# marbl/Winnowmap

Hardware: AMD Instinct MI355X
Metric: mapped Gbp/s (higher is better)
Workload: dtype int8

## Files before the change

### __graft_entry__.py

```python
import os
import sys

ROOT = os.path.dirname(os.path.abspath(__file__))
sys.path.insert(0, ROOT)
sys.path.insert(0, os.path.join(ROOT, "tests"))


def build():
    from winnowmap_amd import build as b
    b.build_gpu(verbose=True)
    b.build_oracle()
    b.build_emu()
    b.build_emu_selfmap()
    b.build_emu_chain()
    b.build_harness()
    import winnowmap_amd
    from winnowmap_amd import gpu
    gpu.lib()


def smoke():
    import numpy as np
    from winnowmap_amd import gpu
    import wmtest as W
    import kswcases
    ctx = gpu.Context(0, 2 << 30)
    cases = kswcases.ont_segments(5, 64)
    sc = gpu.KswScore(2, -4, -1, 4, 2, 24, 1)
    jobs, seqs = gpu.pack_jobs([(c["q"], c["t"], dict(w=c["w"], zdrop=c["zdrop"], end_bonus=c["end_bonus"], flag=c["flag"])) for c in cases])
    res, pool = ctx.ksw_batch(sc, jobs, seqs)
    for i, c in enumerate(cases):
        o = W.o_ksw_extd2(c["q"], c["t"], w=c["w"], zdrop=c["zdrop"], end_bonus=c["end_bonus"], flag=c["flag"])
        assert all(int(res[i][k]) == o[k] for k in W.EZ_FIELDS), (i, res[i], o)
        assert np.array_equal(pool[res[i]["cig_off"]:res[i]["cig_off"] + res[i]["n_cigar"]], o["cigar"]), i
    import ctypes as C
    import tempfile
    from winnowmap_amd import build as b, synth
    tmp = tempfile.mkdtemp()
    ref = synth.make_reference(1, 200000, 5, repeat_frac=0.1)
    fa = os.path.join(tmp, "ref.fa")
    synth.write_fasta(fa, ref)
    km, cnt = synth.repetitive_kmers(ref, 15)
    kf = os.path.join(tmp, "rep.txt")
    synth.write_kmer_list(kf, km, cnt, 15)
    reads, _ = synth.make_reads(ref, 4, 12000, 6, profile="ont", sv_frac=0.25)
    rs = [synth.codes_to_ascii(r) for r in reads]
    idx = gpu.Index(fa, kf, k=15, w=50, n_threads=4)
    idx.upload(ctx)
    m = gpu.Mapper(ctx, idx, "map-ont", gpu.MM_F_CIGAR | gpu.MM_F_OUT_CG)
    text, hits, cigars, first = m.map(["r%d" % i for i in range(len(rs))], rs)
    H = C.CDLL(b.build_harness())
    H.h_index_build.restype = C.c_void_p
    H.h_index_build.argtypes = [C.c_char_p, C.c_char_p, C.c_int, C.c_int, C.c_int]
    H.h_map_many.argtypes = [C.c_void_p, C.c_char_p, C.c_int64, C.c_int, C.POINTER(C.c_char_p), W.i32p, C.c_int, W.i32p, C.c_int, C.POINTER(C.c_int64), W.u32p, C.c_int64, C.POINTER(C.c_int64)]
    hh = H.h_index_build(fa.encode(), kf.encode(), 15, 50, 4)
    n = len(rs)
    ho = np.zeros(16 * 1024, np.int32); co = np.zeros(4000000, np.uint32); hf = (C.c_int64 * (n + 1))(); nc = C.c_int64()
    nh = H.h_map_many(hh, b"map-ont", 0x4 | 0x20, n, (C.c_char_p * n)(*rs), np.array([len(r) for r in rs], np.int32), 2, ho, 1024, hf, co, len(co), C.byref(nc))
    assert nh == len(hits) and nh > 0, (nh, len(hits))
    assert np.array_equal(ho[:16 * nh].reshape(-1, 16), hits) and np.array_equal(co[:nc.value], cigars) and list(hf) == list(first)
    m.close(); idx.close(); ctx.close()
    print("smoke OK: %d ksw alignments and %d end-to-end hits (%d CIGAR ops) bit-exact vs the oracle" % (len(cases), nh, nc.value))


if __name__ == "__main__":
    build()
    if len(sys.argv) > 1 and sys.argv[1] == "smoke":
        smoke()
```

### include/wm_gpu.h

```cpp
#ifndef WM_GPU_H
#define WM_GPU_H
#include <stdint.h>
#include <stddef.h>
#ifdef __cplusplus
extern "C" {
#endif

#define WM_OK        0
#define WM_ENODEV   (-1)
#define WM_EINVAL   (-2)
#define WM_ENOMEM   (-3)
#define WM_EINTERNAL (-4)

typedef struct wm_ctx_s wm_ctx_t;

typedef struct { uint64_t x, y; } wm128_t;

int wm_ctx_create(int device, size_t arena_bytes, wm_ctx_t **out);
void wm_ctx_destroy(wm_ctx_t *ctx);
const char *wm_last_error(void);
const char *wm_build_defines(void);
int wm_device_count(void);
float wm_last_kernel_ms(const wm_ctx_t *ctx);
int wm_ctx_device(const wm_ctx_t *ctx);

typedef struct {
	int8_t match, mismatch, sc_ambi;
	int8_t q, e, q2, e2;
} wm_ksw_score_t;

typedef struct {
	uint32_t q_off, t_off;
	int32_t qlen, tlen;
	int32_t w, zdrop, end_bonus, flag;
} wm_ksw_job_t;

typedef struct {
	int32_t max, zdropped, max_q, max_t, mqe, mqe_t, mte, mte_q, score, reach_end;
	int32_t n_cigar;
	uint32_t cig_off;
} wm_ksw_result_t;

int wm_ksw_batch(wm_ctx_t *ctx, const wm_ksw_score_t *sc, int n_jobs, const wm_ksw_job_t *jobs,
                 const uint8_t *seqs, size_t seqs_bytes,
                 wm_ksw_result_t *results, uint32_t *cigar_pool, size_t cigar_cap, size_t *cigar_used);

typedef struct {
	int64_t qwin_off;
	int32_t qwin_len, q_pos;
	int32_t rid, t_pos;
	int32_t qlen, tlen;
	int32_t w, zdrop, end_bonus, flag;
	int8_t step, has_n, pad[6];
} wm_ksw_pos_t;
int wm_reads_upload(wm_ctx_t *ctx, const uint8_t *codes, size_t n);
int wm_ksw_batch_pos(wm_ctx_t *ctx, const wm_ksw_score_t *sc, int n_jobs, const wm_ksw_pos_t *jobs,
                     wm_ksw_result_t *results, uint32_t *cigar_pool, size_t cigar_cap, size_t *cigar_used);
#define WM_KSW_F_ZDWALK 0x10000
typedef struct { int32_t max_zdrop, t0, t1, q0, q1; } wm_zd_t;
int wm_ksw_batch_pos_zd(wm_ctx_t *ctx, const wm_ksw_score_t *sc, int n_jobs, const wm_ksw_pos_t *jobs,
                        wm_ksw_result_t *results, uint32_t *cigar_pool, size_t cigar_cap, size_t *cigar_used, wm_zd_t *zd);

int wm_debug_stripe_timing(uint64_t *out16, int reset);

int wm_ksw_ll_i16(int qlen, const uint8_t *query, int tlen, const uint8_t *target, const int8_t *mat5x5, int gapo, int gape, int *qe, int *te);

int wm_ksw_exts2_batch(wm_ctx_t *ctx, const wm_ksw_score_t *sc, int noncan, int junc_bonus, int n_jobs, const wm_ksw_job_t *jobs,
                       const uint8_t *seqs, size_t seqs_bytes, const uint8_t *junc,
                       wm_ksw_result_t *results, uint32_t *cigar_pool, size_t cigar_cap, size_t *cigar_used);

typedef struct wm_ksw_dev_batch_s wm_ksw_dev_batch_t;
int wm_ksw_dev_prepare(wm_ctx_t *ctx, const wm_ksw_score_t *sc, int n_jobs, const wm_ksw_job_t *jobs,
                       const uint8_t *seqs, size_t seqs_bytes, wm_ksw_dev_batch_t **out);
int wm_ksw_dev_run(wm_ctx_t *ctx, wm_ksw_dev_batch_t *b);
int wm_ksw_dev_fetch(wm_ctx_t *ctx, wm_ksw_dev_batch_t *b, wm_ksw_result_t *results,
                     uint32_t *cigar_pool, size_t cigar_cap, size_t *cigar_used);
int wm_ksw_dev_stats(const wm_ksw_dev_batch_t *b, uint64_t *cells, uint64_t *tb_bytes, float *dp_ms, float *bt_ms);
void wm_ksw_dev_free(wm_ctx_t *ctx, wm_ksw_dev_batch_t *b);

void wm_ksw_set_routing(int on, int rows4, int rows8);
void wm_ksw_set_chain_routing(int mode, int min_rows_exact, int bp);
void wm_ksw_set_dual(int on);
int wm_ksw_dual_enabled(void);

int wm_ksw_extd2(wm_ctx_t *ctx, int qlen, const uint8_t *query, int tlen, const uint8_t *target, int8_t m,
                 const int8_t *mat, int8_t q, int8_t e, int8_t q2, int8_t e2, int w, int zdrop, int end_bonus,
                 int flag, wm_ksw_result_t *ez, uint32_t **cigar_out);

typedef struct wm_index_s wm_index_t;
int wm_index_build(const char *fasta, const char *kmer_file, int k, int w, int n_threads, wm_index_t **out);
int wm_index_build_gpu(wm_ctx_t *ctx, const char *fasta, const char *kmer_file, int k, int w, int n_threads, wm_index_t **out, double *stats);
int wm_index_build_flag(const char *fasta, const char *kmer_file, int k, int w, int idx_flag, int n_threads, wm_index_t **out);
int wm_index_build_gpu_flag(wm_ctx_t *ctx, const char *fasta, const char *kmer_file, int k, int w, int idx_flag, int n_threads, wm_index_t **out, double *stats);
void wm_index_destroy(wm_index_t *idx);
int wm_index_save(const wm_index_t *idx, const char *path);
int wm_index_load(const char *path, const char *kmer_file, wm_index_t **out);
int wm_index_upload(wm_ctx_t *ctx, const wm_index_t *idx);
int wm_index_read_junc_bed(wm_index_t *idx, const char *path);
int wm_index_add_junc(wm_index_t *idx, int ctg, int n, const int32_t *st, const int32_t *en, const int32_t *strand);
int wm_index_n_seq(const wm_index_t *idx);
const char *wm_index_seq_name(const wm_index_t *idx, int rid);
int wm_index_seq_len(const wm_index_t *idx, int rid);
uint64_t wm_index_n_minimizers(const wm_index_t *idx);
const uint64_t *wm_index_get(const wm_index_t *idx, uint64_t minier, int *n);

int wm_write_repetitive_kmers(const char *fasta, int k, double distinct, const char *out_path, uint64_t *n_out);
int wm_write_repetitive_kmers_gpu(wm_ctx_t *ctx, const char *fasta, int k, double distinct, const char *out_path, uint64_t *n_out, double *stats);
int wm_index_export(const wm_index_t *idx, uint64_t *sizes9, uint32_t *S, uint64_t *hkey, uint64_t *hval, uint64_t *P, uint8_t *bloom,
                    uint64_t *seq_meta, char *names);
int wm_index_import(const uint64_t *sizes9, const uint32_t *S, const uint64_t *hkey, const uint64_t *hval, const uint64_t *P, const uint8_t *bloom,
                    const uint64_t *seq_meta, const char *names, wm_index_t **out);

int wm_sketch_batch(wm_ctx_t *ctx, int n, const uint8_t *seqs, size_t seqs_bytes, const uint64_t *seq_off, const int32_t *len,
                    wm128_t *out, size_t out_cap, uint64_t *out_off, int32_t *counts);
int wm_sketch_set_filter(wm_ctx_t *ctx, const uint8_t *bits, size_t n_bytes, uint64_t table_bits, uint32_t salt0, uint32_t salt1, int k, int w);
int wm_seed_batch(wm_ctx_t *ctx, int n, const wm128_t *mini, const uint64_t *mini_off, const int32_t *n_mini, const int32_t *qlen,
                  int max_occ, int64_t flag, wm128_t *out, size_t out_cap, uint64_t *out_off, int32_t *n_anchors, int32_t *rep_len);
typedef struct { uint32_t lo, eq; } wm_qkey_t;
int wm_index_query_key(const wm_index_t *idx, const char *qname, wm_qkey_t *key);
int wm_seed_batch_keyed(wm_ctx_t *ctx, int n, const wm128_t *mini, const uint64_t *mini_off, const int32_t *n_mini, const int32_t *qlen, const wm_qkey_t *keys,
                        int max_occ, int64_t flag, wm128_t *out, size_t out_cap, uint64_t *out_off, int32_t *n_anchors, int32_t *rep_len);
typedef struct { int32_t max_dist_x, min_dist_x, max_dist_y, bw, max_skip, max_iter, min_cnt, min_sc; float gap_scale;
                 int32_t is_cdna;  } wm_chain_par_t;
int wm_chain_batch(wm_ctx_t *ctx, int n, wm128_t *a, const uint64_t *a_off, const int32_t *n_a, const wm_chain_par_t *par,
                   uint64_t *u, uint64_t *u_off, int32_t *n_u, int32_t *n_v);
typedef struct {
	int64_t seq_off;
	uint64_t stage_off, pre_off;
	int32_t len, n_pre;
	wm_chain_par_t par;
} wm_window_job_t;
typedef struct { int32_t n_anchors, rep_len, n_mini, n_u, n_v; uint32_t u_off, a_off; } wm_window_res_t;
int wm_window_batch(wm_ctx_t *ctx, int n, const wm_window_job_t *jobs, const uint8_t *seqs, size_t seqs_bytes, const wm128_t *pre, size_t n_pre_total,
                    int max_occ, int64_t flag, wm_window_res_t *res, uint64_t *u_pool, size_t u_cap, size_t *u_used, wm128_t *a_pool, size_t a_cap, size_t *a_used);
int wm_window_batch_keyed(wm_ctx_t *ctx, int n, const wm_window_job_t *jobs, const wm_qkey_t *keys, const uint8_t *seqs, size_t seqs_bytes, const wm128_t *pre, size_t n_pre_total,
                          int max_occ, int64_t flag, wm_window_res_t *res, uint64_t *u_pool, size_t u_cap, size_t *u_used, wm128_t *a_pool, size_t a_cap, size_t *a_used);
float wm_last_aux_ms(const wm_ctx_t *ctx);

typedef struct wm_mapper_s wm_mapper_t;
int wm_mapper_create(wm_ctx_t *ctx, const wm_index_t *idx, const char *preset, int64_t flag, wm_mapper_t **out);
void wm_mapper_destroy(wm_mapper_t *m);
int wm_mapper_set_threads(wm_mapper_t *m, int n_threads, size_t arena_bytes_per_group);
int wm_map_reads(wm_mapper_t *m, int n, const char *const *names, const char *const *seqs, const int32_t *lens,
                 const char **text, size_t *text_len, const int32_t **hits, const uint32_t **cigars, const int64_t **hit_first);
#define WM_MAX_SLOTS 4
int wm_map_reads_slot(wm_mapper_t *m, int slot, int n, const char *const *names, const char *const *seqs, const int32_t *lens,
                      const char **text, size_t *text_len, const int32_t **hits, const uint32_t **cigars, const int64_t **hit_first);
int wm_mapper_set_slots(wm_mapper_t *m, int n);
int wm_map_reads_rep_len_defined(const wm_mapper_t *m, int slot, const uint8_t **flags, size_t *n);
int wm_map_file(wm_mapper_t *m, const char *reads_path, const char *out_path, int64_t mini_batch_bases, double *stats);
int wm_index_upload_dev(wm_ctx_t *ctx, const wm_index_t *idx, const void *d_S, const void *d_hkey, const void *d_hval, const void *d_P, const void *d_bloom, int src_device);
int wm_index_upload_peer(wm_ctx_t *dst, const wm_index_t *idx, const wm_ctx_t *src);
int wm_map_file_multi(wm_mapper_t *const *mappers, int n, const char *reads_path, const char *out_path, int64_t mini_batch_bases, double *stats);
int wm_mapper_set_cmdline(wm_mapper_t *m, int argc, const char *const *argv);
int wm_set_cmdline(int argc, const char *const *argv);
typedef struct {
	int64_t flag;
	int32_t seed, sdust_thres, max_qlen;
	int32_t bw, max_gap, max_gap_ref, min_gap_ref, max_frag_len;
	int32_t max_chain_skip, max_chain_iter, min_cnt, min_chain_score;
	float chain_gap_scale;
	int32_t SVaware, SVawareMinReadLength, suffixSampleOffset, min_mapq;
	float min_qcov;
	int32_t minPrefixLength, maxPrefixLength;
	float prefixIncrementFactor;
	int32_t stage2_bw, stage2_zdrop_inv, stage2_max_gap;
	float mask_level;
	int32_t mask_len;
	float pri_ratio;
	int32_t best_n;
	int32_t max_join_long, max_join_short, min_join_flank_sc;
	float min_join_flank_ratio, alt_drop;
	int32_t a, b, q, e, q2, e2, sc_ambi;
	int32_t zdrop, zdrop_inv, end_bonus, min_dp_max, min_ksw_len;
	float max_clip_ratio;
	float mid_occ_frac;
	int32_t min_mid_occ, mid_occ, max_occ;
	int64_t mini_batch_size, max_sw_mat;
	int32_t noncan, junc_bonus;
	int32_t anchor_ext_len, anchor_ext_shift;
} wm_mapopt_t;
int wm_mapopt_preset(const char *preset, wm_mapopt_t *out, int *k, int *w);
int wm_mapper_create_opt(wm_ctx_t *ctx, const wm_index_t *idx, const wm_mapopt_t *opt, wm_mapper_t **out);
int wm_index_build_parts(const char *fasta, const char *kmer_file, int k, int w, int n_threads, uint64_t batch_bases, wm_index_t **out, int cap, int *n_parts);
int wm_map_file_split(wm_ctx_t *ctx, int n_parts, wm_index_t *const *parts, const wm_mapopt_t *opt, int n_threads, const char *reads_path, const char *out_path,
                      int64_t mini_batch_bases, double *stats);
typedef struct wm_split_s wm_split_t;
int wm_split_begin(wm_ctx_t *ctx, const wm_mapopt_t *opt, int k, int w, int n_threads, const char *reads_path, int64_t mini_batch_bases, wm_split_t **out);
int wm_split_add_part(wm_split_t *s, wm_index_t *part);
int wm_split_finish(wm_split_t *s, const char *out_path, double *stats);
void wm_split_abort(wm_split_t *s);
int wm_map_file_split_fasta(wm_ctx_t *ctx, const char *fasta, const char *kmer_file, int k, int w, int build_threads, uint64_t batch_bases, int on_device,
                            const wm_mapopt_t *opt, int n_threads, const char *reads_path, const char *out_path, int64_t mini_batch_bases, double *stats, int *n_parts);

int wm_mapper_set_sam_header(wm_mapper_t *m, int on);
int wm_mapper_stats(const wm_mapper_t *m, uint64_t *out9);
int wm_mapper_kernel_stats(const wm_mapper_t *m, double *out, int cap, int *n_classes);
int wm_ksw_n_classes(void);
int wm_mapper_kernel_union(const wm_mapper_t *m, double since_ms, double *out, int cap, double *now_ms);
int wm_mapper_host_stats(const wm_mapper_t *m, double *out, int cap);
int wm_sam_header(const wm_index_t *idx, int argc, const char *const *argv, const char **text, size_t *text_len);

#ifdef __cplusplus
}
#endif
#endif
```

### winnowmap_amd/build.py

```python
import os
import subprocess
import sys

HERE = os.path.dirname(os.path.abspath(__file__))
ROOT = os.path.dirname(HERE)
CSRC = os.path.join(HERE, "csrc")
LIB = os.path.join(HERE, "libwmgpu.so")
HIPCC = os.environ.get("HIPCC", "/opt/rocm/bin/hipcc")


class _Lock:

    def __init__(self, target):
        self.path = target + ".lock"

    def __enter__(self):
        import fcntl
        self.f = open(self.path, "w")
        fcntl.flock(self.f, fcntl.LOCK_EX)

    def __exit__(self, *a):
        import fcntl
        fcntl.flock(self.f, fcntl.LOCK_UN)
        self.f.close()


def _run_to(target, cmd_for):
    tmp = target + ".tmp%d" % os.getpid()
    try:
        subprocess.check_call(cmd_for(tmp))
        os.replace(tmp, target)
    finally:
        if os.path.exists(tmp):
            os.unlink(tmp)


def _newer(target, sources):
    if not os.path.exists(target):
        return True
    t = os.path.getmtime(target)
    return any(os.path.getmtime(s) > t for s in sources)


HIP_FLAGS = ["--offload-arch=gfx950", "-O3", "-std=c++17", "-ffp-contract=off", "-Wno-unused-value", "-mllvm", "-disable-promote-alloca-to-vector"]


UNITS = ("wm_rt", "wm_ksw", "wm_index", "wm_window", "wm_mapper")


def build_gpu(force=False, verbose=False, out=None):
    global LIB
    if out is not None:
        saved, LIB = LIB, out
        try:
            return build_gpu(force, verbose)
        finally:
            LIB = saved
    srcs = [os.path.join(d, f) for d, _, fs in os.walk(CSRC) for f in fs if ".obj" not in d] + [os.path.join(ROOT, "include", "wm_gpu.h")]
    defines = " ".join(os.environ.get("WM_KERNEL_DEFINES", "").split())
    stamp = LIB + ".defines"
    with _Lock(LIB):
        have = open(stamp).read() if os.path.exists(stamp) else ""
        if not force and not _newer(LIB, srcs) and have == defines:
            return LIB
        defs = ["-D" + d for d in defines.split()] + ['-DWM_BUILD_DEFINES="%s"' % defines]
        objdir = os.path.join(CSRC, ".obj", os.path.basename(LIB))
        os.makedirs(objdir, exist_ok=True)
        cmds = [[HIPCC] + HIP_FLAGS + defs + ["-fPIC", "-c", os.path.join(CSRC, u + ".hip"), "-o", os.path.join(objdir, u + ".o")] for u in UNITS]
        if verbose:
            for c in cmds:
                print(" ".join(c), file=sys.stderr)
        procs = [subprocess.Popen(c) for c in cmds]
        rcs = [p.wait() for p in procs]
        if any(rcs):
            raise subprocess.CalledProcessError(next(r for r in rcs if r), cmds[next(i for i, r in enumerate(rcs) if r)])
        link = lambda out_: [HIPCC, "--offload-arch=gfx950", "-shared", "-fPIC", "-o", out_] + [os.path.join(objdir, u + ".o") for u in UNITS] + ["-lz", "-lpthread"]
        if verbose:
            print(" ".join(link(LIB)), file=sys.stderr)
        _run_to(LIB, link)
        with open(stamp, "w") as f:
            f.write(defines)
    return LIB


def build_oracle():
    with _Lock(os.path.join(ROOT, "oracle", "libwm_oracle.so")):
        subprocess.check_call(["make", "-C", os.path.join(ROOT, "oracle"), "oracle"], stdout=subprocess.DEVNULL)
        if os.path.exists("/root/reference/src/map.c"):
            subprocess.check_call(["make", "-C", os.path.join(ROOT, "oracle"), "ref", "-j8"], stdout=subprocess.DEVNULL)
            if os.path.exists(LIB):
                subprocess.check_call(["make", "-C", os.path.join(ROOT, "oracle"), "wm", "subst", "-j8"], stdout=subprocess.DEVNULL)


def build_emu(defines=()):
    emu = os.path.join(ROOT, "tests", "simt_emu")
    tag = "".join("_" + "".join(ch if ch.isalnum() else "_" for ch in d) for d in defines)
    out = os.path.join(emu, "libwm_emu%s.so" % tag)
    srcs = [os.path.join(emu, f) for f in ("emu_driver.cpp", "simt.h")] + [os.path.join(CSRC, f) for f in os.listdir(CSRC) if f.endswith(".h")]
    with _Lock(out):
        if _newer(out, srcs):
            _run_to(out, lambda o: ["g++", "-O1", "-std=c++17", "-fPIC", "-shared", "-ffp-contract=off", "-Wno-unknown-pragmas"] +
                    ["-D" + d for d in defines] + ["-I" + emu, "-I" + CSRC, "-o", o, os.path.join(emu, "emu_driver.cpp")])
    return out


def build_emu_selfmap():
    emu = os.path.join(ROOT, "tests", "simt_emu")
    out = os.path.join(emu, "libwm_emu_selfmap.so")
    srcs = [os.path.join(emu, f) for f in ("emu_selfmap.cpp", "simt.h")] + \
           [os.path.join(CSRC, f) for f in ("seedchain_kernel.h", "window_kernel.h", "wm_internal.h", os.path.join("host", "wm_names.h"))]
    with _Lock(out):
        if _newer(out, srcs):
            _run_to(out, lambda o: ["g++", "-O1", "-std=c++17", "-fPIC", "-shared", "-ffp-contract=off", "-Wno-unknown-pragmas",
                                    "-I" + emu, "-I" + CSRC, "-o", o, os.path.join(emu, "emu_selfmap.cpp")])
    return out


def build_emu_stripe(defines=()):
    emu = os.path.join(ROOT, "tests", "simt_emu")
    tag = "".join("_" + "".join(ch if ch.isalnum() else "_" for ch in d) for d in defines)
    out = os.path.join(emu, "libwm_emu_stripe%s.so" % tag)
    srcs = [os.path.join(emu, f) for f in ("emu_stripe.cpp", "simt.h")] + \
           [os.path.join(CSRC, f) for f in ("ksw_stripe_kernel.h", "ksw_packed_kernel.h", "ksw_kernel.h", "ksw_plan.h")]
    with _Lock(out):
        if _newer(out, srcs):
            _run_to(out, lambda o: ["g++", "-O1", "-std=c++17", "-fPIC", "-shared", "-pthread", "-ffp-contract=off", "-Wno-unknown-pragmas"] +
                    ["-D" + d for d in defines] + ["-I" + emu, "-I" + CSRC, "-o", o, os.path.join(emu, "emu_stripe.cpp")])
    return out


def build_emu_chain(defines=()):
    emu = os.path.join(ROOT, "tests", "simt_emu")
    tag = "".join("_" + "".join(ch if ch.isalnum() else "_" for ch in d) for d in defines)
    out = os.path.join(emu, "libwm_emu_chain%s.so" % tag)
    srcs = [os.path.join(emu, f) for f in ("emu_chain.cpp", "simt.h")] + \
           [os.path.join(CSRC, f) for f in ("ksw_chain_kernel.h", "ksw_stripe_kernel.h", "ksw_packed_kernel.h", "ksw_kernel.h", "ksw_plan.h")]
    with _Lock(out):
        if _newer(out, srcs):
            _run_to(out, lambda o: ["g++", "-O1", "-std=c++17", "-fPIC", "-shared", "-pthread", "-ffp-contract=off", "-Wno-unknown-pragmas"] +
                    ["-D" + d for d in defines] + ["-I" + emu, "-I" + CSRC, "-o", o, os.path.join(emu, "emu_chain.cpp")])
    return out


def build_harness():
    hd = os.path.join(ROOT, "tests", "host_harness")
    out = os.path.join(hd, "libwm_harness.so")
    srcs = [os.path.join(hd, "harness.cpp"), os.path.join(ROOT, "oracle", "wm_oracle.c")] + \
           [os.path.join(CSRC, "host", f) for f in os.listdir(os.path.join(CSRC, "host"))]
    with _Lock(out):
        if _newer(out, srcs):
            _run_to(out, lambda o: ["g++", "-std=c++17", "-O2", "-g", "-ffp-contract=off", "-fPIC", "-shared", "-o", o,
                                    os.path.join(hd, "harness.cpp"), os.path.join(ROOT, "oracle", "wm_oracle.c"), "-lz", "-pthread"])
    return out


if __name__ == "__main__":
    build_gpu(force="--force" in sys.argv, verbose=True)
    build_oracle()
    build_emu()
    build_emu_selfmap()
    build_emu_stripe()
    build_emu_chain()
    build_harness()
```

### winnowmap_amd/csrc/wm_ksw.hip

```cpp
#include "wm_rt.h"
#include "simt.h"
#include "ksw_kernel.h"
#include "ksw_packed_kernel.h"
#include "ksw_packed_multi_kernel.h"
#include "ksw_dual_kernel.h"
#include "ksw_stripe_kernel.h"
#include "ksw_chain_kernel.h"
#include "ksw_exts2_kernel.h"
#include "cigar_walk.h"
#include "reads2bit.h"

#ifndef WM_OCC_HINT
#define WM_OCC_HINT 1
#endif
template <int BP, bool CLIP, bool HASN, bool EXACT>
__global__ __launch_bounds__(64, (WM_OCC_HINT && BP == 8 && CLIP && EXACT) ? 4 : 1) void ksw_dpp_kernel(wm_ksw_score_t sc, const wm_ksw_djob_t *__restrict__ jobs,
                                                      const int *__restrict__ order, const uint8_t *__restrict__ seqs,
                                                      uint8_t *__restrict__ tb, wm_ksw_dres_t *__restrict__ res)
{
	if constexpr (EXACT || CLIP || BP >= 16) WM_SETPRIO(2);
	const int j = order[blockIdx.x];
	wmk::ksw_dp_packed<BP, CLIP, HASN, EXACT>(sc, jobs[j], seqs, tb, res + j);
}

__global__ __launch_bounds__(64) void ksw_generic_kernel(wm_ksw_score_t sc, const wm_ksw_djob_t *__restrict__ jobs, const int *__restrict__ order,
                                                          const uint8_t *__restrict__ seqs, uint8_t *__restrict__ tb, uint8_t *scratch,
                                                          const uint64_t *__restrict__ scratch_off, wm_ksw_dres_t *__restrict__ res)
{
	WM_SETPRIO(3);
	const int j = order[blockIdx.x];
	const wm_ksw_djob_t jb = jobs[j];
	const int T = (jb.tlen + 15) / 16 * 16;
	signed char *mem = (signed char*)(scratch + scratch_off[blockIdx.x]);
	int *Hm = (int*)(mem + (size_t)8 * T);
	wmk::ksw_dp_generic<true>(sc, jb, seqs, tb, mem, Hm, res + j);
}

template <int K, int WN>
__global__ __launch_bounds__(64 * WM_KSW_BLK_NWV) void ksw_block_kernel(wm_ksw_score_t sc, const wm_ksw_djob_t *__restrict__ jobs, const int *__restrict__ order,
                                                                         const uint8_t *__restrict__ seqs, uint8_t *__restrict__ tb, wm_ksw_dres_t *__restrict__ res, int seq_cap,
                                                                         int *gstate, const uint64_t *__restrict__ gstate_off)
{
	WM_SETPRIO(3);
	extern __shared__ __attribute__((aligned(16))) unsigned char smem[];
	constexpr bool GLOBAL = WN == 0;
	const int j = order[blockIdx.x];
	const wm_ksw_djob_t jb = jobs[j];
	const int wn = GLOBAL ? (int)wm_ksw_blk3_wn(jb.tlen) : WN;
	int *W0 = GLOBAL ? gstate + gstate_off[blockIdx.x] : (int*)smem, *W1 = W0 + wn, *Hm = W1 + wn;
	int *pub = GLOBAL ? (int*)smem : Hm + wn;
	uint8_t *sq = (uint8_t*)(pub + WM_KSW_BLK_PUB);
	const int qpad = (jb.qlen + 15) & ~15;
	if (qpad + jb.tlen <= seq_cap) {
		uint8_t *st = sq + qpad;
		for (int i = threadIdx.x; i < jb.qlen; i += blockDim.x) sq[i] = seqs[jb.q_off + i];
		for (int i = threadIdx.x; i < jb.tlen; i += blockDim.x) st[i] = seqs[jb.t_off + i];
		__syncthreads();
		wmk::ksw_dp_block<WM_KSW_BLK_NWV, K, GLOBAL>(sc, jb, sq, st, tb, W0, W1, Hm, wn, pub, res + j);
	} else
		wmk::ksw_dp_block<WM_KSW_BLK_NWV, K, GLOBAL>(sc, jb, seqs + jb.q_off, seqs + jb.t_off, tb, W0, W1, Hm, wn, pub, res + j);
}

template <int BP, int NWV, bool CLIP = true, bool HASN = true>
__global__ __launch_bounds__(64 * NWV) void ksw_pmulti_kernel(wm_ksw_score_t sc, const wm_ksw_djob_t *__restrict__ jobs, const int *__restrict__ order,
                                                                         const uint8_t *__restrict__ seqs, uint8_t *__restrict__ tb, wm_ksw_dres_t *__restrict__ res, int seq_cap)
{
	WM_SETPRIO(3);
	extern __shared__ __attribute__((aligned(16))) unsigned char smem[];
	typedef wmk::ksw_pmulti_lds<BP, NWV> L;
	int *lds = (int*)smem;
	uint8_t *sq = (uint8_t*)(lds + L::INTS);
	const int j = order[blockIdx.x];
	const wm_ksw_djob_t jb = jobs[j];
	const int qpad = (jb.qlen + 15) & ~15;
	if (qpad + jb.tlen <= seq_cap) {
		uint8_t *st = sq + qpad;
		for (int i = threadIdx.x; i < jb.qlen; i += blockDim.x) sq[i] = seqs[jb.q_off + i];
		for (int i = threadIdx.x; i < jb.tlen; i += blockDim.x) st[i] = seqs[jb.t_off + i];
		__syncthreads();
		if (jb.flag & KSW_F_APPROX_MAX) wmk::ksw_dp_pmulti<BP, NWV, CLIP, HASN, false>(sc, jb, sq, st, tb, lds, res + j);
		else wmk::ksw_dp_pmulti<BP, NWV, CLIP, HASN, true>(sc, jb, sq, st, tb, lds, res + j);
	} else {
		const uint8_t *qp = seqs + jb.q_off, *tp = seqs + jb.t_off;
		if (jb.flag & KSW_F_APPROX_MAX) wmk::ksw_dp_pmulti<BP, NWV, CLIP, HASN, false>(sc, jb, qp, tp, tb, lds, res + j);
		else wmk::ksw_dp_pmulti<BP, NWV, CLIP, HASN, true>(sc, jb, qp, tp, tb, lds, res + j);
	}
}

template <int BP, int NWV, bool CLIP, bool HASN>
__global__ __launch_bounds__(64 * NWV) void ksw_stripe_kernel(wm_ksw_score_t sc, const wm_ksw_djob_t *__restrict__ jobs, const int *__restrict__ order,
                                                               const uint8_t *__restrict__ seqs, uint8_t *__restrict__ tb, wm_ksw_dres_t *__restrict__ res)
{
	WM_SETPRIO(WM_STRIPE_PRIO);
	__shared__ int lds[wmk::ksw_stripe_lds<BP, NWV>::INTS];
	const int j = order[blockIdx.x];
	const wm_ksw_djob_t jb = jobs[j];
	if (jb.flag & KSW_F_APPROX_MAX) wmk::ksw_dp_stripe<BP, NWV, CLIP, HASN, false>(sc, jb, seqs, tb, lds, res + j);
	else wmk::ksw_dp_stripe<BP, NWV, CLIP, HASN, true>(sc, jb, seqs, tb, lds, res + j);
}

template <int BP, bool CLIP, bool HASN, bool EXACT>
__global__ __launch_bounds__(64, (WM_OCC_HINT && BP == 2 && EXACT) ? 4 : 1) void ksw_chain_kernel(wm_ksw_score_t sc, const wm_ksw_djob_t *__restrict__ jobs, const int *__restrict__ order,
                                                        const uint8_t *__restrict__ seqs, uint8_t *__restrict__ tb, wm_ksw_dres_t *__restrict__ res,
                                                        const uint4 *__restrict__ cmap, int *ticket, wm_mbox_t *mail)
{
	WM_SETPRIO(WM_STRIPE_PRIO);
	__shared__ int tbs[wm_chain_box::GROUP * 32 * BP];
	int tk = 0;
	if (threadIdx.x == 0) tk = atomicAdd(ticket, 1);
	tk = __builtin_amdgcn_readfirstlane(tk);
	const uint4 m = cmap[tk];
	const int j = order[m.x];
	const wm_ksw_djob_t jb = jobs[j];
	wm_mbox_t *mb = mail + (size_t)m.z * 16;
	wmk::ksw_dp_chain<BP, CLIP, HASN, EXACT>(sc, jb, seqs, tb, mb, (int)m.w, (int)m.y, tbs, res + j);
}

__global__ __launch_bounds__(256) void ksw_reset_kernel(int n, const wm_ksw_djob_t *__restrict__ jobs, wm_ksw_dres_t *__restrict__ res)
{
	const int j = blockIdx.x * 256 + threadIdx.x;
	if (j >= n || jobs[j].klass >= 0) return;
	wm_ksw_dres_t z;
	z.max = 0; z.zdropped = 0; z.max_q = z.max_t = z.mqe_t = z.mte_q = -1; z.score = z.mqe = z.mte = KSW_NEG_INF; z.reach_end = 0; z.n_cigar = 0; z.bt_i = z.bt_j = -1;
	res[j] = z;
}

__global__ __launch_bounds__(64) void ksw_expand_kernel(const wm_ksw_djob_t *__restrict__ jobs, const wm_ksw_dsrc_t *__restrict__ src,
                                                         const uint64_t *__restrict__ reads_pk, const uint64_t *__restrict__ reads_nm, const uint32_t *__restrict__ S,
                                                         uint8_t *__restrict__ seqs)
{
	WM_SETPRIO(1);
	const int j = blockIdx.x;
	const wm_ksw_djob_t jb = jobs[j];
	if (jb.klass < 0) return;
	const wm_ksw_dsrc_t sr = src[j];
	const int64_t L = sr.qwin_len;
	uint8_t *q = seqs + jb.q_off, *t = seqs + jb.t_off;
	for (int i = threadIdx.x; i < jb.qlen; i += 64) {
		const int64_t p = (int64_t)sr.q_pos + (int64_t)i * sr.step;
		uint8_t c = 4;
		if (p >= 0 && p < L) c = (uint8_t)wmk::rd2_code(reads_pk, reads_nm, (long long)(sr.qwin_off + p));
		else if (p >= L && p < 2 * L) { c = (uint8_t)wmk::rd2_code(reads_pk, reads_nm, (long long)(sr.qwin_off + (2 * L - 1 - p))); c = c < 4 ? 3 - c : 4; }
		q[i] = c;
	}
	for (int i = threadIdx.x; i < jb.tlen; i += 64) {
		const int64_t p = sr.t_base + (int64_t)i * sr.step;
		t[i] = (uint8_t)(S[p >> 3] >> ((p & 7) << 2) & 0xf);
	}
}

__global__ __launch_bounds__(64) void ksw_backtrack_kernel(int n, const wm_ksw_djob_t *__restrict__ jobs, const uint8_t *__restrict__ tb,
                                                            wm_ksw_dres_t *__restrict__ res, uint32_t *__restrict__ cig_scratch, int *__restrict__ err)
{
	WM_SETPRIO(3);
	const int j = blockIdx.x * 64 + threadIdx.x;
	if (j >= n) return;
	wm_ksw_dres_t r = res[j];
	int nc = 0;
	if (r.bt_i == KSW_BT_WATCHDOG) atomicMax(err, 2);
	if (r.bt_i >= 0) {
		nc = wmk::ksw_backtrack_thread(jobs[j], tb, r.bt_i, r.bt_j, cig_scratch + jobs[j].cig_off, jobs[j].cig_cap);
		if (nc < 0) { atomicMax(err, 1); nc = 0; }
	}
	res[j].n_cigar = nc;
}

__global__ __launch_bounds__(64) void ksw_backtrack_coop_kernel(int n, const wm_ksw_djob_t *__restrict__ jobs, const uint8_t *__restrict__ tb,
                                                                 wm_ksw_dres_t *__restrict__ res, uint32_t *__restrict__ cig_scratch, int *__restrict__ err)
{
	WM_SETPRIO(3);
	__shared__ uint8_t tile[KSW_BT_ROWS * 64];
	const int j = blockIdx.x;
	const int bt_i = res[j].bt_i, bt_j = res[j].bt_j;
	int nc = 0;
	if (bt_i == KSW_BT_WATCHDOG && threadIdx.x == 0) atomicMax(err, 2);
	if (bt_i >= 0) {
		nc = wmk::ksw_backtrack_wave(jobs[j], tb, bt_i, bt_j, cig_scratch + jobs[j].cig_off, jobs[j].cig_cap, tile);
		if (nc < 0) { if (threadIdx.x == 0) atomicMax(err, 1); nc = 0; }
	}
	if (threadIdx.x == 0) res[j].n_cigar = nc;
}

__global__ __launch_bounds__(1024) void ksw_scan_kernel(int n, const wm_ksw_dres_t *__restrict__ res, uint32_t *__restrict__ off, uint32_t *__restrict__ total)
{
	WM_SETPRIO(3);
	__shared__ uint32_t part[1024];
	const int tid = threadIdx.x, per = (n + 1023) / 1024, b = tid * per, e = b + per < n ? b + per : n;
	uint32_t s = 0;
	for (int i = b; i < e; ++i) s += (uint32_t)res[i].n_cigar;
	part[tid] = s;
	__syncthreads();
	if (tid == 0) {
		uint32_t acc = 0;
		for (int i = 0; i < 1024; ++i) { uint32_t t = part[i]; part[i] = acc; acc += t; }
		*total = acc;
	}
	__syncthreads();
	s = part[tid];
	for (int i = b; i < e; ++i) { off[i] = s; s += (uint32_t)res[i].n_cigar; }
}

__global__ __launch_bounds__(64) void ksw_gather_kernel(const wm_ksw_djob_t *__restrict__ jobs, const wm_ksw_dres_t *__restrict__ res,
                                                         const uint32_t *__restrict__ off, const uint32_t *__restrict__ cig_scratch,
                                                         uint32_t *__restrict__ pool, uint32_t pool_cap)
{
	WM_SETPRIO(3);
	const int j = blockIdx.x, n = res[j].n_cigar;
	const uint32_t *src = cig_scratch + jobs[j].cig_off;
	const bool rev = (jobs[j].flag & KSW_F_REV_CIGAR) != 0;
	for (int i = threadIdx.x; i < n; i += 64) {
		const uint32_t dst = off[j] + (uint32_t)i;
		if (dst < pool_cap) pool[dst] = src[rev ? i : n - 1 - i];
	}
}

__global__ __launch_bounds__(64) void ksw_zdwalk_kernel(int n, wm_ksw_score_t sc, const wm_ksw_djob_t *__restrict__ jobs, const wm_ksw_dres_t *__restrict__ res,
                                                         const uint32_t *__restrict__ off, const uint32_t *__restrict__ pool, const uint8_t *__restrict__ seqs,
                                                         wm_zd_t *__restrict__ zd)
{
	WM_SETPRIO(3);
	const int j = blockIdx.x * 64 + threadIdx.x;
	if (j >= n) return;
	wm_zd_t z = { 0, -1, -1, -1, -1 };
	if ((jobs[j].flag & WM_KSW_F_ZDWALK) && !(jobs[j].flag & KSW_F_REV_CIGAR))
		wm_zdrop_walk(seqs + jobs[j].q_off, seqs + jobs[j].t_off, pool + off[j], res[j].n_cigar, sc.match, sc.mismatch, sc.sc_ambi, sc.q, sc.e, &z);
	zd[j] = z;
}

struct wm_ksw_dev_batch_s {
	int n_jobs;
	wm_ksw_score_t sc, sc_in;
	wm_zd_t *d_zd = 0;
	std::vector<wm_ksw_djob_t> jobs;
	std::vector<int> order[WM_KSW_NCLASS];
	std::vector<int> ord;
	std::vector<int> degenerate;
	std::vector<std::string> dumped;
	uint8_t *d_gscratch; uint64_t *d_goff; std::vector<uint64_t> goff;
	uint8_t *d_b3state; uint64_t *d_b3off; std::vector<uint64_t> b3off;
	std::vector<uint4> cmap[WM_KSW_NCLASS - WM_KSW_CHAIN][2]; uint4 *d_cmap[WM_KSW_NCLASS - WM_KSW_CHAIN][2]; wm_mbox_t *d_mail = 0; size_t mail_words = 0; int *d_tickets = 0;
	wm_ksw_djob_t *d_jobs; int *d_order; uint8_t *d_seqs, *d_tb; wm_ksw_dres_t *d_res; uint32_t *d_cig, *d_off, *d_total, *d_pool; int *d_err;
	size_t pool_cap, arena_mark, slab_bytes;
	uint64_t cells, tb_bytes;
	uint64_t class_cells[WM_KSW_NCLASS];
	float dp_ms, bt_ms;
	uint32_t total_ops;
	int h_err;
};

template <int NC>
__global__ __launch_bounds__(64, (WM_OCC_HINT && NC == 8) ? 4 : 1) void ksw_dual_kernel(wm_ksw_score_t sc, const wm_ksw_djob_t *__restrict__ jobs, const int *__restrict__ order, int n,
                                                      const uint8_t *__restrict__ seqs, uint8_t *__restrict__ tb, wm_ksw_dres_t *__restrict__ res)
{
	const int g = blockIdx.x, jA = order[2 * g];
	const bool hasB = 2 * g + 1 < n;
	const int jB = hasB ? order[2 * g + 1] : jA;
	wmk::ksw_dp_dual<NC>(sc, jobs[jA], jobs[jB], hasB, seqs, tb, res + jA, res + jB);
}
static std::atomic<int> g_dual(-1);
static int ksw_dual_on()
{
	if (g_dual.load(std::memory_order_relaxed) < 0) g_dual = getenv("WM_KSW_DUAL") && atoi(getenv("WM_KSW_DUAL")) != 0;
	return g_dual.load(std::memory_order_relaxed);
}
extern "C" void wm_ksw_set_dual(int on) { g_dual = on ? 1 : 0; }
extern "C" int wm_ksw_dual_enabled(void) { return ksw_dual_on(); }

template <int BP> static void launch_dpp(int variant, int n, hipStream_t s, const wm_ksw_score_t &sc, const wm_ksw_djob_t *jobs, const int *order,
                                         const uint8_t *seqs, uint8_t *tb, wm_ksw_dres_t *res)
{
	dim3 g(n), b(64);
	const bool exact = variant & 4, clip = (variant & 2) || (variant & 1), hasn = variant & 1;
	if (exact) {
		if (hasn) hipLaunchKernelGGL((ksw_dpp_kernel<BP, true, true, true>), g, b, 0, s, sc, jobs, order, seqs, tb, res);
		else if (clip) hipLaunchKernelGGL((ksw_dpp_kernel<BP, true, false, true>), g, b, 0, s, sc, jobs, order, seqs, tb, res);
		else hipLaunchKernelGGL((ksw_dpp_kernel<BP, false, false, true>), g, b, 0, s, sc, jobs, order, seqs, tb, res);
	} else {
		if (hasn) hipLaunchKernelGGL((ksw_dpp_kernel<BP, true, true, false>), g, b, 0, s, sc, jobs, order, seqs, tb, res);
		else if (clip) hipLaunchKernelGGL((ksw_dpp_kernel<BP, true, false, false>), g, b, 0, s, sc, jobs, order, seqs, tb, res);
		else if (BP <= 8 && ksw_dual_on()) hipLaunchKernelGGL((ksw_dual_kernel<(BP <= 8 ? 2 * BP : 16)>), dim3((n + 1) / 2), b, 0, s, sc, jobs, order, n, seqs, tb, res);
		else hipLaunchKernelGGL((ksw_dpp_kernel<BP, false, false, false>), g, b, 0, s, sc, jobs, order, seqs, tb, res);
	}
}

static std::atomic<int> g_stripe_on(-1), g_stripe_rows4(-1), g_stripe_rows8(-1), g_stripe_wide16(0);
static int stripe_min_rows(int bp)
{
	if (g_stripe_on.load(std::memory_order_relaxed) < 0) {
		g_stripe_rows4 = getenv("WM_KSW_STRIPE_ROWS4") ? std::max(0, atoi(getenv("WM_KSW_STRIPE_ROWS4"))) : 0;
		g_stripe_rows8 = getenv("WM_KSW_STRIPE_ROWS8") ? std::max(0, atoi(getenv("WM_KSW_STRIPE_ROWS8"))) : 4096;
		g_stripe_wide16 = getenv("WM_KSW_STRIPE16") ? atoi(getenv("WM_KSW_STRIPE16")) & 3 : 1;
		g_stripe_on = !(getenv("WM_KSW_STRIPE") && atoi(getenv("WM_KSW_STRIPE")) == 0);
	}
	return !g_stripe_on.load(std::memory_order_relaxed) ? 0 : bp == 4 ? g_stripe_rows4.load(std::memory_order_relaxed) : bp == 8 ? g_stripe_rows8.load(std::memory_order_relaxed) : 1;
}
extern "C" void wm_ksw_set_routing(int on, int rows4, int rows8)
{
	stripe_min_rows(0);
	if (on >= 0) { g_stripe_on = on != 0; g_stripe_wide16 = on == 2 ? 3 : on == 3 ? 0 : 1; }
	if (rows4 >= 0) g_stripe_rows4 = rows4;
	if (rows8 >= 0) g_stripe_rows8 = rows8;
}

template <int BP, int NWV> static void launch_stripe(int variant, int n, hipStream_t s, const wm_ksw_score_t &sc, const wm_ksw_djob_t *jobs, const int *order,
                                                     const uint8_t *seqs, uint8_t *tb, wm_ksw_dres_t *res)
{
	dim3 g(n), b(64 * NWV);
	if (variant & 1) hipLaunchKernelGGL((ksw_stripe_kernel<BP, NWV, true, true>), g, b, 0, s, sc, jobs, order, seqs, tb, res);
	else if (variant & 2) hipLaunchKernelGGL((ksw_stripe_kernel<BP, NWV, true, false>), g, b, 0, s, sc, jobs, order, seqs, tb, res);
	else hipLaunchKernelGGL((ksw_stripe_kernel<BP, NWV, false, false>), g, b, 0, s, sc, jobs, order, seqs, tb, res);
}

template <int BP, bool EXACT> static void launch_chain(int variant, int n, hipStream_t s, const wm_ksw_score_t &sc, const wm_ksw_djob_t *jobs, const int *order,
                                                       const uint8_t *seqs, uint8_t *tb, wm_ksw_dres_t *res, const uint4 *cmap, int *ticket, wm_mbox_t *mail)
{
	dim3 g(n), b(64);
	if (variant & 1) hipLaunchKernelGGL((ksw_chain_kernel<BP, true, true, EXACT>), g, b, 0, s, sc, jobs, order, seqs, tb, res, cmap, ticket, mail);
	else if (variant & 2) hipLaunchKernelGGL((ksw_chain_kernel<BP, true, false, EXACT>), g, b, 0, s, sc, jobs, order, seqs, tb, res, cmap, ticket, mail);
	else hipLaunchKernelGGL((ksw_chain_kernel<BP, false, false, EXACT>), g, b, 0, s, sc, jobs, order, seqs, tb, res, cmap, ticket, mail);
}
static std::atomic<int> g_chain_mode(-1), g_chain_rows(2048), g_chain_geom(0);
static int chain_mode()
{
	if (g_chain_mode.load(std::memory_order_relaxed) < 0) {
		g_chain_rows = getenv("WM_KSW_CHAIN_ROWS") ? std::max(1, atoi(getenv("WM_KSW_CHAIN_ROWS"))) : 2048;
		g_chain_geom = getenv("WM_KSW_CHAIN_BP") && atoi(getenv("WM_KSW_CHAIN_BP")) == 4 ? 1 : 0;
		g_chain_mode = getenv("WM_KSW_CHAIN") ? atoi(getenv("WM_KSW_CHAIN")) & 7 : 1;
	}
	return g_chain_mode.load(std::memory_order_relaxed);
}
extern "C" void wm_ksw_set_chain_routing(int mode, int min_rows_exact, int bp)
{
	chain_mode();
	if (mode >= 0) g_chain_mode = mode & 7;
	if (min_rows_exact > 0) g_chain_rows = min_rows_exact;
	if (bp == 2 || bp == 4) g_chain_geom = bp == 4 ? 1 : 0;
}

static int ksw_prepare_impl(wm_ctx_t *c, const wm_ksw_score_t *sc_in, int n_jobs, const wm_ksw_job_t *jobs, const uint8_t *seqs, size_t seqs_bytes,
                            const wm_ksw_pos_t *pos, wm_ksw_dev_batch_t **out)
{
	*out = 0;
	if (!c) return set_err(WM_EINVAL, "null context");
	if (n_jobs < 0) return set_err(WM_EINVAL, "n_jobs < 0");
	wm_ksw_score_t sc = *sc_in;
	if (!wm_ksw_score_ok(&sc)) return set_err(WM_EINVAL, "unsupported scoring parameters (need match>0, mismatch<0, sc_ambi<=0, q,e,q2>0, e2>=0, (q+e)+(q2+e2)<=127 as src/options.c:166-176)");
	if (sc.q2 + sc.e2 < sc.q + sc.e) { int8_t t = sc.q; sc.q = sc.q2; sc.q2 = t; t = sc.e; sc.e = sc.e2; sc.e2 = t; }
	if (pos && (!c->d_S || c->seq_len.empty())) return set_err(WM_EINVAL, "position jobs need wm_index_upload on this context");
	if (pos && !c->d_reads) return set_err(WM_EINVAL, "position jobs need wm_reads_upload on this context");
	HIPCHK(hipSetDevice(c->device));
	wm_ksw_dev_batch_t *b = new wm_ksw_dev_batch_t();
	b->n_jobs = n_jobs; b->sc = sc; b->sc_in = *sc_in; b->cells = b->tb_bytes = 0; b->dp_ms = b->bt_ms = 0; b->total_ops = 0; b->h_err = 0;
	memset(b->class_cells, 0, sizeof(b->class_cells));
	b->arena_mark = c->arena_used;
	b->jobs.resize(n_jobs);
	UBuf<wm_ksw_dsrc_t> dsrc(pos ? n_jobs : 0, c);
	size_t slab_lo = 0, slab_bytes = 0;
	int bad0 = -1;
	if (pos) {
		uint64_t tot = 0;
		for (int i = 0; i < n_jobs; ++i) {
			const wm_ksw_pos_t &s = pos[i];
			wm_ksw_djob_t &d = b->jobs[i];
			const uint64_t ql = s.qlen > 0 ? s.qlen : 0, tl = s.tlen > 0 ? s.tlen : 0;
			d.q_off = (uint32_t)tot; d.t_off = (uint32_t)(tot + ql);
			tot += ql + tl;
		}
		std::atomic<int> badp(-1);
		WM_SITE("ksw.positions");
		wm::parallel_for(c->host_threads, (size_t)n_jobs, [&](size_t i) {
			const wm_ksw_pos_t &s = pos[i];
			memset(&dsrc[i], 0, sizeof(dsrc[i]));
			if (s.qlen <= 0 || s.tlen <= 0) return;
			const int64_t t_last = (int64_t)s.t_pos + (int64_t)(s.tlen - 1) * s.step;
			if ((s.step != 1 && s.step != -1) || s.rid < 0 || (size_t)s.rid >= c->seq_len.size() || s.t_pos < 0 || t_last < 0 ||
			    (uint32_t)s.t_pos >= c->seq_len[s.rid] || (uint64_t)t_last >= c->seq_len[s.rid] ||
			    s.qwin_off < 0 || s.qwin_len < 0 || (uint64_t)s.qwin_off + (uint64_t)s.qwin_len > c->reads_bytes) { badp = (int)i; return; }
			dsrc[i].qwin_off = s.qwin_off; dsrc[i].qwin_len = s.qwin_len; dsrc[i].q_pos = s.q_pos; dsrc[i].step = s.step; dsrc[i].pad = 0;
			dsrc[i].t_base = (int64_t)c->seq_off[s.rid] + s.t_pos;
		});
		if (badp >= 0) bad0 = badp;
		if (tot >= ((uint64_t)1 << 32)) { delete b; return set_err(WM_ENOMEM, "batch holds %.1f GB of sequence (limit 4 GB per batch)", tot / 1073741824.0); }
		slab_bytes = (size_t)tot;
	} else {
		size_t lo = seqs_bytes, hi = 0;
		for (int i = 0; i < n_jobs; ++i) {
			const wm_ksw_job_t &s = jobs[i];
			if (s.qlen <= 0 || s.tlen <= 0) continue;
			if ((size_t)s.q_off + s.qlen > seqs_bytes || (size_t)s.t_off + s.tlen > seqs_bytes) { if (bad0 < 0) bad0 = i; continue; }
			lo = std::min(lo, (size_t)std::min(s.q_off, s.t_off));
			hi = std::max(hi, std::max((size_t)s.q_off + s.qlen, (size_t)s.t_off + s.tlen));
		}
		if (hi > lo) { slab_lo = lo; slab_bytes = hi - lo; }
	}
	if (bad0 >= 0) { delete b; return set_err(WM_EINVAL, pos ? "job %d: operand positions outside the resident reads / reference" : "job %d: sequence offsets outside seqs", bad0); }
	const int n_sc = sc.sc_ambi == 0 ? -sc.e2 : sc.sc_ambi;
	int min_sc = sc.mismatch < n_sc ? sc.mismatch : n_sc;
	if (sc.sc_ambi < min_sc) min_sc = sc.sc_ambi;
	const bool never = -min_sc > 2 * (sc.q + sc.e);
	uint64_t tb_off = 0, cig_off = 0;
	std::vector<uint64_t> cells(n_jobs, 0), bands(n_jobs, 0);
	std::atomic<int> bad(-1);
	WM_SITE("ksw.classify");
	wm::parallel_for(c->host_threads, (size_t)n_jobs, [&](size_t i) {
		wm_ksw_djob_t &d = b->jobs[i];
		int32_t qlen, tlen, w, zdrop, end_bonus, flag;
		uint32_t q_off = d.q_off, t_off = d.t_off;
		if (pos) { const wm_ksw_pos_t &s = pos[i]; qlen = s.qlen; tlen = s.tlen; w = s.w; zdrop = s.zdrop; end_bonus = s.end_bonus; flag = s.flag; }
		else { const wm_ksw_job_t &s = jobs[i]; qlen = s.qlen; tlen = s.tlen; w = s.w; zdrop = s.zdrop; end_bonus = s.end_bonus; flag = s.flag; q_off = s.q_off; t_off = s.t_off; }
		memset(&d, 0, sizeof(d));
		d.qlen = qlen; d.tlen = tlen; d.w = w; d.zdrop = zdrop; d.end_bonus = end_bonus; d.flag = flag;
		if (flag & (0x01 | 0x04 | 0x10 | 0x100 | 0x200 | 0x400)) { bad = (int)i; d.klass = -1; return; }
		if (qlen <= 0 || tlen <= 0 || never) { d.klass = -1; return; }
		const int has_n = pos ? (pos[i].has_n != 0) : (wm_ksw_has_n(seqs + q_off, qlen) | wm_ksw_has_n(seqs + t_off, tlen));
		d.q_off = pos ? q_off : (uint32_t)(q_off - slab_lo); d.t_off = pos ? t_off : (uint32_t)(t_off - slab_lo);
		int n_col;
		d.klass = wm_ksw_classify(qlen, tlen, w, has_n, flag, &n_col);
		static const bool merge_p8x = !(getenv("WM_KSW_MERGE_P8X") && atoi(getenv("WM_KSW_MERGE_P8X")) == 0);
		if (merge_p8x && (d.klass & ~7) == WM_KSW_P8 && (d.klass & 4) && !(d.klass & 2)) d.klass |= 2;
		if (stripe_min_rows(0)) d.klass = wm_ksw_route(d.klass, n_col, qlen, tlen, w, has_n, stripe_min_rows(4), stripe_min_rows(8), g_stripe_wide16.load(std::memory_order_relaxed));
		d.klass = wm_ksw_route_chain(d.klass, qlen, tlen, w, has_n, flag, chain_mode(), g_chain_rows.load(std::memory_order_relaxed), g_chain_geom.load(std::memory_order_relaxed));
		d.n_col = n_col;
		cells[i] = wm_ksw_cells(qlen, tlen, w, &bands[i]);
	});
	if (bad >= 0) {
		const int i = bad;
		delete b;
		return set_err(WM_EINVAL, "job %d: KSW_EZ_SCORE_ONLY/GENERIC_SC/APPROX_DROP/SPLICE flags are not used by the mapper (src/align.c) and not supported", i);
	}
	for (int i = 0; i < n_jobs; ++i) {
		wm_ksw_djob_t &d = b->jobs[i];
		if (d.klass < 0) { b->degenerate.push_back(i); continue; }
		d.tb_off = tb_off;
		const uint64_t rows = (uint64_t)d.qlen + d.tlen - 1;
		tb_off += (rows * d.n_col + 15) & ~(uint64_t)15;
		d.cig_off = (uint32_t)cig_off; d.cig_cap = d.qlen + d.tlen + 2;
		cig_off += d.cig_cap;
		b->cells += bands[i]; b->tb_bytes += cells[i];
		b->class_cells[d.klass] += bands[i];
		b->order[d.klass].push_back(i);
	}
	{
		auto size_key = [&](int j) { const uint64_t v = cells[j] | 1; const int e = 63 - __builtin_clzll(v); return 2 * e + (int)(e > 0 ? (v >> (e - 1)) & 1 : 0); };
		std::vector<int> tmp;
		for (int k = 0; k < WM_KSW_NCLASS; ++k) {
			std::vector<int> &o = b->order[k];
			if (o.size() < 2) continue;
			int cnt[130];
			memset(cnt, 0, sizeof(cnt));
			for (int j : o) ++cnt[size_key(j)];
			int pos_[130], acc = 0;
			for (int kk = 129; kk >= 0; --kk) { pos_[kk] = acc; acc += cnt[kk]; }
			tmp.resize(o.size());
			for (int j : o) tmp[pos_[size_key(j)]++] = j;
			o.swap(tmp);
		}
	}
	size_t chain_mw = 0;
	bool chain_any = false;
	for (int kc = 0; kc < WM_KSW_NCLASS - WM_KSW_CHAIN; ++kc) {
		const int sw = 128 * wm_ksw_chain_bp[kc >> 2];
		const std::vector<int> &o = b->order[WM_KSW_CHAIN + kc];
		b->d_cmap[kc][0] = b->d_cmap[kc][1] = 0;
		for (size_t jo = 0; jo < o.size(); ++jo) {
			const wm_ksw_djob_t &d = b->jobs[o[jo]];
			const int nwv = wm_chain_nwv(d.n_col, d.tlen, sw);
			std::vector<uint4> &cm = b->cmap[kc][(d.flag & KSW_F_APPROX_MAX) ? 0 : 1];
			for (int wv = 0; wv < nwv; ++wv) cm.push_back(make_uint4((unsigned)jo, (unsigned)wv, (unsigned)(chain_mw / 16), (unsigned)nwv));
			chain_mw += ((size_t)wm_chain_box::words(nwv) + 15) & ~(size_t)15;
			chain_any = true;
		}
	}
	const size_t nj = n_jobs > 0 ? n_jobs : 1;
	auto al256 = [](size_t x) { return (x + 255) & ~(size_t)255; };
	const size_t o_ord = al256(nj * sizeof(wm_ksw_djob_t)), o_src = o_ord + al256(nj * sizeof(int));
	size_t o_cm[WM_KSW_NCLASS - WM_KSW_CHAIN][2], tab_bytes = o_src + (pos ? al256(nj * sizeof(wm_ksw_dsrc_t)) : 0);
	for (int kc = 0; kc < WM_KSW_NCLASS - WM_KSW_CHAIN; ++kc)
		for (int e = 0; e < 2; ++e) { o_cm[kc][e] = tab_bytes; tab_bytes += al256(b->cmap[kc][e].size() * sizeof(uint4)); }
	uint8_t *d_tab = (uint8_t*)arena_take(c, tab_bytes);
	b->d_jobs = (wm_ksw_djob_t*)d_tab;
	b->d_order = d_tab ? (int*)(d_tab + o_ord) : 0;
	for (int kc = 0; kc < WM_KSW_NCLASS - WM_KSW_CHAIN && d_tab; ++kc)
		for (int e = 0; e < 2; ++e) if (!b->cmap[kc][e].empty()) b->d_cmap[kc][e] = (uint4*)(d_tab + o_cm[kc][e]);
	b->d_res = (wm_ksw_dres_t*)arena_take(c, al256(nj * sizeof(wm_ksw_dres_t)) + nj * 4 + 64);
	b->d_off = b->d_res ? (uint32_t*)((uint8_t*)b->d_res + al256(nj * sizeof(wm_ksw_dres_t))) : 0;
	b->d_err = (int*)arena_take(c, 64);
	b->d_total = b->d_err ? (uint32_t*)(b->d_err + 1) : 0;
	bool any_zd = false;
	for (int i = 0; i < n_jobs && !any_zd; ++i) any_zd = (b->jobs[i].flag & WM_KSW_F_ZDWALK) != 0;
	b->d_zd = any_zd ? (wm_zd_t*)arena_take(c, nj * sizeof(wm_zd_t)) : 0;
	b->d_seqs = (uint8_t*)arena_take(c, slab_bytes + 64);
	b->slab_bytes = slab_bytes;
	wm_ksw_dsrc_t *d_src = pos && d_tab ? (wm_ksw_dsrc_t*)(d_tab + o_src) : 0;
	b->d_cig = (uint32_t*)arena_take(c, (cig_off + 16) * 4);
	b->pool_cap = cig_off + 16;
	b->d_pool = (uint32_t*)arena_take(c, b->pool_cap * 4);
	b->d_tb = (uint8_t*)arena_take(c, tb_off + 64);
	{
		uint64_t go = 0;
		for (int j : b->order[WM_KSW_GENERIC]) { const uint64_t T = ((uint64_t)b->jobs[j].tlen + 15) / 16 * 16; b->goff.push_back(go); go += 12 * T + 256; }
		b->d_gscratch = (uint8_t*)arena_take(c, go + 256);
		b->d_goff = (uint64_t*)arena_take(c, b->goff.size() * 8 + 64);
		if (!b->d_gscratch || !b->d_goff) b->d_tb = 0;
		uint64_t so = 0;
		for (int j : b->order[WM_KSW_BLOCK3]) { b->b3off.push_back(so); so += 3 * wm_ksw_blk3_wn(b->jobs[j].tlen); }
		b->d_b3state = (uint8_t*)arena_take(c, so * 4 + 256);
		b->d_b3off = (uint64_t*)arena_take(c, b->b3off.size() * 8 + 64);
		if (!b->d_b3state || !b->d_b3off) b->d_tb = 0;
	}
	if (chain_any) {
		b->mail_words = chain_mw;
		b->d_mail = (wm_mbox_t*)arena_take(c, chain_mw * 8 + 256);
		b->d_tickets = (int*)arena_take(c, 64 * sizeof(int));
		if (!b->d_mail || !b->d_tickets) b->d_tb = 0;
	}
	if (!b->d_jobs || !b->d_order || !b->d_res || !b->d_off || !b->d_total || !b->d_err || !b->d_seqs || (any_zd && !b->d_zd) || (pos && !d_src) || !b->d_cig || !b->d_pool || !b->d_tb) {
		c->arena_used = b->arena_mark;
		delete b;
		return set_err(WM_ENOMEM, "batch needs %.1f MB of traceback + buffers; arena is %.1f MB", (tb_off + cig_off * 8 + slab_bytes) / 1048576.0, c->arena_bytes / 1048576.0);
	}
	b->ord.clear();
	b->ord.reserve(nj);
	for (int k = 0; k < WM_KSW_NCLASS; ++k) b->ord.insert(b->ord.end(), b->order[k].begin(), b->order[k].end());
	UBuf<uint8_t> ptab(tab_bytes, c);
	if (n_jobs) memcpy(ptab.data(), b->jobs.data(), (size_t)n_jobs * sizeof(wm_ksw_djob_t));
	if (!b->ord.empty()) memcpy(ptab.data() + o_ord, b->ord.data(), b->ord.size() * sizeof(int));
	if (pos && n_jobs > 0) memcpy(ptab.data() + o_src, dsrc.data(), (size_t)n_jobs * sizeof(wm_ksw_dsrc_t));
	for (int kc = 0; kc < WM_KSW_NCLASS - WM_KSW_CHAIN; ++kc)
		for (int e = 0; e < 2; ++e)
			if (!b->cmap[kc][e].empty()) memcpy(ptab.data() + o_cm[kc][e], b->cmap[kc][e].data(), b->cmap[kc][e].size() * sizeof(uint4));
	HIPCHK(hipMemcpyAsync(d_tab, ptab.data(), tab_bytes, hipMemcpyHostToDevice, c->stream));
	if (pos) {
		if (n_jobs > 0) hipLaunchKernelGGL(ksw_expand_kernel, dim3(n_jobs), dim3(64), 0, c->stream, b->d_jobs, d_src, c->d_reads, c->d_reads_nm, c->d_S, b->d_seqs);
	} else if (slab_bytes) HIPCHK(hipMemcpyAsync(b->d_seqs, seqs + slab_lo, slab_bytes, hipMemcpyHostToDevice, c->stream));
	if (!b->goff.empty()) HIPCHK(hipMemcpyAsync(b->d_goff, b->goff.data(), b->goff.size() * 8, hipMemcpyHostToDevice, c->stream));
	if (!b->b3off.empty()) HIPCHK(hipMemcpyAsync(b->d_b3off, b->b3off.data(), b->b3off.size() * 8, hipMemcpyHostToDevice, c->stream));
	HIPCHK(ctx_sync(c));
	*out = b;
	return WM_OK;
}

extern "C" int wm_ksw_dev_prepare(wm_ctx_t *c, const wm_ksw_score_t *sc_in, int n_jobs, const wm_ksw_job_t *jobs,
                                  const uint8_t *seqs, size_t seqs_bytes, wm_ksw_dev_batch_t **out)
{
	return ksw_prepare_impl(c, sc_in, n_jobs, jobs, seqs, seqs_bytes, 0, out);
}

int reads_alloc(wm_ctx_t *c, size_t cap)
{
	const size_t pkw = cap / 32 + 2, nmw = cap / 64 + 2;
	c->d_reads = 0; c->d_reads_nm = 0; c->reads_cap = 0;
	if (hipMalloc((void**)&c->d_reads, (pkw + nmw) * 8) != hipSuccess) { (void)hipGetLastError(); c->d_reads = 0; return set_err(WM_ENOMEM, "cannot allocate %zu bytes for the resident reads", (pkw + nmw) * 8); }
	c->d_reads_nm = c->d_reads + pkw;
	c->reads_cap = cap;
	return WM_OK;
}
extern "C" int wm_reads_upload(wm_ctx_t *c, const uint8_t *codes, size_t n)
{
	if (!c || (n && !codes)) return set_err(WM_EINVAL, "null argument");
	HIPCHK(hipSetDevice(c->device));
	if (!c->owns_reads) { c->d_reads = 0; c->d_reads_nm = 0; c->reads_cap = 0; }
	if (n + 256 > c->reads_cap) {
		if (c->d_reads) HIPCHK(hipFree(c->d_reads));
		c->d_reads = 0; c->d_reads_nm = 0; c->reads_cap = 0;
		const size_t cap = (n + n / 8 + (1 << 20) + 255) & ~(size_t)255;
		const int rc = reads_alloc(c, cap);
		if (rc) return rc;
	}
	c->owns_reads = true;
	std::vector<uint64_t> pk(wm_pk_words(n)), nm(wm_nm_words(n));
	wm_pack_codes(codes, n, pk.data(), nm.data());
	HIPCHK(hipMemcpy(c->d_reads, pk.data(), pk.size() * 8, hipMemcpyHostToDevice));
	HIPCHK(hipMemcpy(c->d_reads_nm, nm.data(), nm.size() * 8, hipMemcpyHostToDevice));
	c->reads_bytes = n;
	return WM_OK;
}

static bool pmulti_lean() { static const bool v = !(getenv("WM_KSW_PMULTI_LEAN") && atoi(getenv("WM_KSW_PMULTI_LEAN")) == 0); return v; }
static int ksw_pmulti_level() { const char *e = getenv("WM_KSW_PMULTI"); return e ? atoi(e) : 2; }

extern "C" int wm_ksw_dev_run(wm_ctx_t *c, wm_ksw_dev_batch_t *b)
{
	HIPCHK(hipSetDevice(c->device));
	const int n = b->n_jobs;
	if (n == 0) return WM_OK;
	HIPCHK(hipMemsetAsync(b->d_err, 0, 4, c->stream));
	if (b->d_mail) {
		HIPCHK(hipMemsetAsync(b->d_mail, 0xff, b->mail_words * 8, c->stream));
		HIPCHK(hipMemsetAsync(b->d_tickets, 0, 64 * sizeof(int), c->stream));
	}
	if (!b->degenerate.empty()) hipLaunchKernelGGL(ksw_reset_kernel, dim3((n + 255) / 256), dim3(256), 0, c->stream, n, b->d_jobs, b->d_res);
	HIPCHK(hipEventRecord(c->ev[0], c->stream));
	int off = 0;
	static const bool trace_k = getenv("WM_TRACE_KSW") != 0;
	auto class_done = [&](int k, double t0) {
		if (!trace_k) return;
		hipStreamSynchronize(c->stream);
		const std::vector<int> &o = b->order[k];
		const wm_ksw_djob_t &big = b->jobs[o[0]];
		fprintf(stderr, "[ksw class %2d] jobs %zu  %.2f ms  largest q=%d t=%d w=%d flag=0x%x n_col=%d\n", k, o.size(), now_ms() - t0, big.qlen, big.tlen, big.w, big.flag, big.n_col);
	};
	int n_nonempty = 0, used_mask = 0, rr = 0;
	for (int k = 0; k < WM_KSW_NCLASS; ++k) n_nonempty += !b->order[k].empty();
	static const int n_side = std::max(0, std::min(4, getenv("WM_SIDE_STREAMS") ? atoi(getenv("WM_SIDE_STREAMS")) : 3));
	const bool fan = n_nonempty > 1 && !trace_k && n_side > 0;
	if (fan) HIPCHK(hipEventRecord(c->kev[4], c->stream));
	hipStream_t ks = c->stream;
	hipStream_t side[4] = {0, 0, 0, 0};
	int pool_lo = 0, pool_n = c->n_side_pool, wclass = 0;
	if (c->side_pool && c->n_side_pool >= 6) {
		static const long heavy_units = getenv("WM_KSW_HEAVY_UNITS") ? atol(getenv("WM_KSW_HEAVY_UNITS")) : 8192, huge_units = getenv("WM_KSW_HUGE_UNITS") ? atol(getenv("WM_KSW_HUGE_UNITS")) : 131072;
		static int split_l = -1, split_h = -1;
		if (split_l < 0) { int a, h; side_split(c->n_side_pool, &a, &h); split_h = h; split_l = a; }
		if (split_l > 0 && split_h > 0 && split_l + split_h < c->n_side_pool) {
			long mx = 0;
			for (const wm_ksw_djob_t &d : b->jobs) {
				if (d.klass < 0) continue;
				long w_ = d.w < 0 ? std::max(d.qlen, d.tlen) : d.w, nn = std::min(d.qlen, d.tlen);
				if (nn > w_ + 1) nn = w_ + 1;
				mx = std::max(mx, ((long)d.qlen + d.tlen) * ((nn + 127) / 128 + 1));
			}
			wclass = huge_units > 0 && mx > huge_units ? 2 : heavy_units > 0 && mx > heavy_units ? 1 : 0;
			pool_lo = wclass == 0 ? 0 : wclass == 1 ? split_l : split_l + split_h;
			pool_n = wclass == 0 ? split_l : wclass == 1 ? split_h : c->n_side_pool - split_l - split_h;
		}
	}
	const int n_use = c->side_pool ? std::min(n_side, pool_n) : n_side;
	if (fan && n_use > 0) {
		if (c->side_pool) { const unsigned b0 = c->side_next[wclass].fetch_add((unsigned)n_use); for (int i = 0; i < n_use; ++i) side[i] = c->side_pool[pool_lo + (int)((b0 + (unsigned)i) % (unsigned)pool_n)]; }
		else for (int i = 0; i < n_use; ++i) { if (!c->kstream[i]) HIPCHK(hipStreamCreateWithFlags(&c->kstream[i], hipStreamNonBlocking)); side[i] = c->kstream[i]; }
	}
	auto next_stream = [&]() {
		if (!fan || n_use <= 0) return;
		const int si = rr++ % n_use;
		ks = side[si];
		if (!(used_mask >> si & 1)) { hipStreamWaitEvent(ks, c->kev[4], 0); used_mask |= 1 << si; }
	};
	static const bool class_events = !(getenv("WM_KSW_CLASS_EVENTS") && atoi(getenv("WM_KSW_CLASS_EVENTS")) == 0);
	int offs[WM_KSW_NCLASS + 1];
	offs[0] = 0;
	for (int k = 0; k < WM_KSW_NCLASS; ++k) offs[k + 1] = offs[k] + (int)b->order[k].size();
	int lorder[WM_KSW_NCLASS], nl = 0;
	lorder[nl++] = WM_KSW_GENERIC; lorder[nl++] = WM_KSW_BLOCK3; lorder[nl++] = WM_KSW_BLOCK2; lorder[nl++] = WM_KSW_BLOCK;
	for (int k = WM_KSW_NCLASS - 1; k >= WM_KSW_STRIPE; --k) lorder[nl++] = k;
	for (int k = WM_KSW_BLOCK - 1; k >= 0; --k) lorder[nl++] = k;
	for (int li = 0; li < nl; ++li) {
		const int k = lorder[li];
		const int nk = (int)b->order[k].size();
		if (nk == 0) continue;
		off = offs[k];
		next_stream();
		const double tk0 = trace_k ? now_ms() : 0;
		if (class_events) hipEventRecord(c->cev[k][0], ks);
		struct Done { decltype(class_done) &f; int k; double t; hipEvent_t e; hipStream_t s; bool on; ~Done() { if (on) hipEventRecord(e, s); f(k, t); } } done_guard{ class_done, k, tk0, c->cev[k][1], ks, class_events };
		if (k == WM_KSW_BLOCK || k == WM_KSW_BLOCK2 || k == WM_KSW_BLOCK3) {
			const size_t fixed = (size_t)WM_KSW_BLK_PUB * 4;
			if (k == WM_KSW_BLOCK || k == WM_KSW_BLOCK2) {
				const int seq_cap = 64 * 1024;
				if (k == WM_KSW_BLOCK) {
					const size_t lds = (size_t)wmk::ksw_pmulti_lds<4, 8>::INTS * 4 + seq_cap;
					HIPCHK(hipFuncSetAttribute((const void*)ksw_pmulti_kernel<4, 8>, hipFuncAttributeMaxDynamicSharedMemorySize, (int)lds));
					hipLaunchKernelGGL((ksw_pmulti_kernel<4, 8>), dim3(nk), dim3(64 * 8), lds, ks, b->sc, b->d_jobs, b->d_order + off, b->d_seqs, b->d_tb, b->d_res, seq_cap);
				} else {
					const size_t lds = (size_t)wmk::ksw_pmulti_lds<8, 8>::INTS * 4 + seq_cap;
					HIPCHK(hipFuncSetAttribute((const void*)ksw_pmulti_kernel<8, 8>, hipFuncAttributeMaxDynamicSharedMemorySize, (int)lds));
					hipLaunchKernelGGL((ksw_pmulti_kernel<8, 8>), dim3(nk), dim3(64 * 8), lds, ks, b->sc, b->d_jobs, b->d_order + off, b->d_seqs, b->d_tb, b->d_res, seq_cap);
				}
			} else {
				const size_t lds = fixed + WM_KSW_BLK3_SEQ_LDS;
				HIPCHK(hipFuncSetAttribute((const void*)ksw_block_kernel<WM_KSW_BLK2_K, 0>, hipFuncAttributeMaxDynamicSharedMemorySize, (int)lds));
				hipLaunchKernelGGL((ksw_block_kernel<WM_KSW_BLK2_K, 0>), dim3(nk), dim3(64 * WM_KSW_BLK_NWV), lds, ks, b->sc, b->d_jobs, b->d_order + off, b->d_seqs, b->d_tb, b->d_res, (int)WM_KSW_BLK3_SEQ_LDS, (int*)b->d_b3state, b->d_b3off);
			}
			continue;
		}
		if (k >= WM_KSW_CHAIN) {
			const int kc = k - WM_KSW_CHAIN, var = kc & 3;
			for (int e = 1; e >= 0; --e) {
				const int nw = (int)b->cmap[kc][e].size();
				if (!nw) continue;
				if (wm_ksw_chain_bp[kc >> 2] == 2) {
					if (e) launch_chain<2, true>(var, nw, ks, b->sc, b->d_jobs, b->d_order + off, b->d_seqs, b->d_tb, b->d_res, b->d_cmap[kc][e], b->d_tickets + 2 * kc + e, b->d_mail);
					else launch_chain<2, false>(var, nw, ks, b->sc, b->d_jobs, b->d_order + off, b->d_seqs, b->d_tb, b->d_res, b->d_cmap[kc][e], b->d_tickets + 2 * kc + e, b->d_mail);
				} else {
					if (e) launch_chain<4, true>(var, nw, ks, b->sc, b->d_jobs, b->d_order + off, b->d_seqs, b->d_tb, b->d_res, b->d_cmap[kc][e], b->d_tickets + 2 * kc + e, b->d_mail);
					else launch_chain<4, false>(var, nw, ks, b->sc, b->d_jobs, b->d_order + off, b->d_seqs, b->d_tb, b->d_res, b->d_cmap[kc][e], b->d_tickets + 2 * kc + e, b->d_mail);
				}
			}
			continue;
		}
		if (k >= WM_KSW_STRIPE) {
			const int var = (k - WM_KSW_STRIPE) & 3;
			static const char *dump_dir = getenv("WM_KSW_DUMP");
			if (dump_dir) {
				static std::atomic<int> seq(0);
				std::vector<uint8_t> hs(b->slab_bytes + 64);
				hipStreamSynchronize(c->stream);
				hipMemcpy(hs.data(), b->d_seqs, b->slab_bytes, hipMemcpyDeviceToHost);
				char path[512];
				snprintf(path, sizeof(path), "%s/stripe_%d_%d.bin", dump_dir, (int)getpid(), seq++);
				if (FILE *fp = fopen(path, "wb")) {
					const int32_t hdr[4] = { k, nk, (int32_t)sizeof(wm_ksw_djob_t), (int32_t)sizeof(wm_ksw_score_t) };
					fwrite(hdr, 4, 4, fp); fwrite(&b->sc, sizeof(b->sc), 1, fp);
					for (int j : b->order[k]) {
						const wm_ksw_djob_t &d = b->jobs[j];
						fwrite(&d, sizeof(d), 1, fp); fwrite(hs.data() + d.q_off, 1, d.qlen, fp); fwrite(hs.data() + d.t_off, 1, d.tlen, fp);
					}
					fclose(fp);
					b->dumped.push_back(path);
				}
			}
			switch ((k - WM_KSW_STRIPE) >> 2) {
			case 0: launch_stripe<2, 4>(var, nk, ks, b->sc, b->d_jobs, b->d_order + off, b->d_seqs, b->d_tb, b->d_res); break;
			case 1: launch_stripe<2, 8>(var, nk, ks, b->sc, b->d_jobs, b->d_order + off, b->d_seqs, b->d_tb, b->d_res); break;
			case 2: launch_stripe<4, 8>(var, nk, ks, b->sc, b->d_jobs, b->d_order + off, b->d_seqs, b->d_tb, b->d_res); break;
			case 4: launch_stripe<1, 16>(var, nk, ks, b->sc, b->d_jobs, b->d_order + off, b->d_seqs, b->d_tb, b->d_res); break;
			case 5: launch_stripe<2, 16>(var, nk, ks, b->sc, b->d_jobs, b->d_order + off, b->d_seqs, b->d_tb, b->d_res); break;
			default: launch_stripe<8, 8>(var, nk, ks, b->sc, b->d_jobs, b->d_order + off, b->d_seqs, b->d_tb, b->d_res); break;
			}
			continue;
		}
		if (k == WM_KSW_GENERIC) {
			hipLaunchKernelGGL(ksw_generic_kernel, dim3(nk), dim3(64), 0, ks, b->sc, b->d_jobs, b->d_order + off, b->d_seqs, b->d_tb, b->d_gscratch, b->d_goff, b->d_res);
			continue;
		}
		switch (k & ~7) {
		case WM_KSW_P4: launch_dpp<4>(k & 7, nk, ks, b->sc, b->d_jobs, b->d_order + off, b->d_seqs, b->d_tb, b->d_res); break;
		case WM_KSW_P8: launch_dpp<8>(k & 7, nk, ks, b->sc, b->d_jobs, b->d_order + off, b->d_seqs, b->d_tb, b->d_res); break;
		default:
			if (ksw_pmulti_level() >= 2) {
				const int seq_cap = 32 * 1024;
				const size_t lds = (size_t)wmk::ksw_pmulti_lds<4, 4>::INTS * 4 + seq_cap;
				auto go = [&](auto kern) -> int {
					HIPCHK(hipFuncSetAttribute((const void*)kern, hipFuncAttributeMaxDynamicSharedMemorySize, (int)lds));
					hipLaunchKernelGGL(kern, dim3(nk), dim3(64 * 4), lds, ks, b->sc, b->d_jobs, b->d_order + off, b->d_seqs, b->d_tb, b->d_res, seq_cap);
					return WM_OK;
				};
				int rc_;
				if (!pmulti_lean()) rc_ = go(ksw_pmulti_kernel<4, 4, true, true>);
				else if ((k & 2) && (k & 1)) rc_ = go(ksw_pmulti_kernel<4, 4, true, true>);
				else if (k & 2) rc_ = go(ksw_pmulti_kernel<4, 4, true, false>);
				else if (k & 1) rc_ = go(ksw_pmulti_kernel<4, 4, false, true>);
				else rc_ = go(ksw_pmulti_kernel<4, 4, false, false>);
				if (rc_) return rc_;
			} else
				launch_dpp<16>(k & 7, nk, ks, b->sc, b->d_jobs, b->d_order + off, b->d_seqs, b->d_tb, b->d_res);
			break;
		}
	}
	for (int si = 0; si < 4; ++si)
		if (used_mask >> si & 1) { HIPCHK(hipEventRecord(c->kev[si], side[si])); HIPCHK(hipStreamWaitEvent(c->stream, c->kev[si], 0)); }
	HIPCHK(hipEventRecord(c->ev[1], c->stream));
	if (getenv("WM_KSW_COOP_BT") && atoi(getenv("WM_KSW_COOP_BT")) > 0)
		hipLaunchKernelGGL(ksw_backtrack_coop_kernel, dim3(n), dim3(64), 0, c->stream, n, b->d_jobs, b->d_tb, b->d_res, b->d_cig, b->d_err);
	else
		hipLaunchKernelGGL(ksw_backtrack_kernel, dim3((n + 63) / 64), dim3(64), 0, c->stream, n, b->d_jobs, b->d_tb, b->d_res, b->d_cig, b->d_err);
	hipLaunchKernelGGL(ksw_scan_kernel, dim3(1), dim3(1024), 0, c->stream, n, b->d_res, b->d_off, b->d_total);
	hipLaunchKernelGGL(ksw_gather_kernel, dim3(n), dim3(64), 0, c->stream, b->d_jobs, b->d_res, b->d_off, b->d_cig, b->d_pool, (uint32_t)b->pool_cap);
	if (b->d_zd) hipLaunchKernelGGL(ksw_zdwalk_kernel, dim3((n + 63) / 64), dim3(64), 0, c->stream, n, b->sc_in, b->d_jobs, b->d_res, b->d_off, b->d_pool, b->d_seqs, b->d_zd);
	HIPCHK(hipEventRecord(c->ev[2], c->stream));
	HIPCHK(hipGetLastError());
	int *h_small = c->pin_small ? c->pin_small : &b->h_err;
	uint32_t *h_total = c->pin_small ? (uint32_t*)(c->pin_small + 1) : &b->total_ops;
	if (c->pin_small) HIPCHK(hipMemcpyAsync(h_small, b->d_err, 8, hipMemcpyDeviceToHost, c->stream));
	else { HIPCHK(hipMemcpyAsync(h_small, b->d_err, 4, hipMemcpyDeviceToHost, c->stream)); HIPCHK(hipMemcpyAsync(h_total, b->d_total, 4, hipMemcpyDeviceToHost, c->stream)); }
	HIPCHK(ctx_sync(c));
	b->h_err = *h_small; b->total_ops = *h_total;
	for (const std::string &f : b->dumped) unlink(f.c_str());
	b->dumped.clear();
	HIPCHK(hipEventElapsedTime(&b->dp_ms, c->ev[0], c->ev[1]));
	HIPCHK(hipEventElapsedTime(&b->bt_ms, c->ev[1], c->ev[2]));
	c->last_ms = b->dp_ms + b->bt_ms;
	for (int k = 0; k < WM_KSW_NCLASS && class_events; ++k)
		if (!b->order[k].empty()) {
			float ms = 0;
			if (hipEventElapsedTime(&ms, c->cev[k][0], c->cev[k][1]) == hipSuccess) {
				c->k_ms[k] += ms; c->k_cells[k] += b->class_cells[k]; c->k_launches[k] += 1;
				float t0 = 0;
				if (hipEvent_t base = device_base_event(c->device)) if (hipEventElapsedTime(&t0, base, c->cev[k][0]) == hipSuccess) {
					std::lock_guard<std::mutex> lk(c->iv_mu);
					if (c->k_iv[k].size() > 100000) c->k_iv[k].erase(c->k_iv[k].begin(), c->k_iv[k].begin() + 50000);
					c->k_iv[k].push_back(std::make_pair(t0, t0 + ms));
				}
			}
		}
	if (b->h_err == 2) return set_err(WM_EINTERNAL, "a stripe-pipelined / chained-workgroup alignment kernel gave up waiting for a neighbouring wavefront (watchdog, ksw_stripe_kernel.h, ksw_chain_kernel.h); WM_KSW_CHAIN=0 / WM_KSW_STRIPE=0 route around them");
	if (b->h_err) return set_err(WM_EINTERNAL, "cigar slot overflow in backtrack");
	return WM_OK;
}

extern "C" int wm_ksw_dev_fetch(wm_ctx_t *c, wm_ksw_dev_batch_t *b, wm_ksw_result_t *results, uint32_t *cigar_pool, size_t cigar_cap, size_t *cigar_used)
try {
	HIPCHK(hipSetDevice(c->device));
	const int n = b->n_jobs;
	if (cigar_used) *cigar_used = b->total_ops;
	if (n == 0) return WM_OK;
	const size_t off_at = (size_t)((uint8_t*)b->d_off - (uint8_t*)b->d_res);
	UBuf<uint8_t> ro(off_at + (size_t)n * 4, c);
	const wm_ksw_dres_t *res = (const wm_ksw_dres_t*)ro.data();
	const uint32_t *off = (const uint32_t*)(ro.data() + off_at);
	if (b->total_ops > cigar_cap) return set_err(WM_ENOMEM, "cigar_pool too small: need %u ops", b->total_ops);
	HIPCHK(hipMemcpyAsync(ro.data(), b->d_res, off_at + (size_t)n * 4, hipMemcpyDeviceToHost, c->stream));
	if (b->total_ops) HIPCHK(hipMemcpyAsync(cigar_pool, b->d_pool, (size_t)b->total_ops * 4, hipMemcpyDeviceToHost, c->stream));
	HIPCHK(ctx_sync(c));
	WM_SITE("ksw.results");
	wm::parallel_for(c->host_threads, (size_t)n, [&](size_t i) {
		wm_ksw_result_t &o = results[i];
		const wm_ksw_dres_t &r = res[i];
		o.max = r.max; o.zdropped = r.zdropped; o.max_q = r.max_q; o.max_t = r.max_t; o.mqe = r.mqe; o.mqe_t = r.mqe_t;
		o.mte = r.mte; o.mte_q = r.mte_q; o.score = r.score; o.reach_end = r.reach_end; o.n_cigar = r.n_cigar; o.cig_off = off[i];
	});
	return WM_OK;
}
catch (const std::bad_alloc &) { return set_err(WM_ENOMEM, "out of host memory"); }

extern "C" int wm_ksw_dev_stats(const wm_ksw_dev_batch_t *b, uint64_t *cells, uint64_t *tb_bytes, float *dp_ms, float *bt_ms)
{
	if (cells) *cells = b->cells;
	if (tb_bytes) *tb_bytes = b->tb_bytes;
	if (dp_ms) *dp_ms = b->dp_ms;
	if (bt_ms) *bt_ms = b->bt_ms;
	return WM_OK;
}

extern "C" void wm_ksw_dev_free(wm_ctx_t *c, wm_ksw_dev_batch_t *b)
{
	if (!b) return;
	if (c && c->arena_used >= b->arena_mark) c->arena_used = b->arena_mark;
	delete b;
}

static int ksw_fetch_zd(wm_ctx_t *c, wm_ksw_dev_batch_t *b, wm_zd_t *out)
{
	const int n = b->n_jobs;
	if (!b->d_zd) { for (int i = 0; i < n; ++i) out[i] = wm_zd_t{ 0, -1, -1, -1, -1 }; return WM_OK; }
	if (n == 0) return WM_OK;
	HIPCHK(hipSetDevice(c->device));
	UBuf<wm_zd_t> z(n, c);
	HIPCHK(hipMemcpyAsync(z.data(), b->d_zd, (size_t)n * sizeof(wm_zd_t), hipMemcpyDeviceToHost, c->stream));
	HIPCHK(ctx_sync(c));
	memcpy(out, z.data(), (size_t)n * sizeof(wm_zd_t));
	return WM_OK;
}

static int ksw_batch_impl(wm_ctx_t *c, const wm_ksw_score_t *sc, int n_jobs, const wm_ksw_job_t *jobs, const uint8_t *seqs, size_t seqs_bytes, const wm_ksw_pos_t *pos,
                          wm_ksw_result_t *results, uint32_t *cigar_pool, size_t cigar_cap, size_t *cigar_used, wm_zd_t *zd = 0)
{
	if (!c) return set_err(WM_EINVAL, "null context");
	size_t used = 0;
	int i0 = 0;
	float kms = 0;
	const size_t budget = (size_t)(c->arena_bytes * 0.8);
	while (i0 < n_jobs || (n_jobs == 0 && i0 == 0)) {
		int i1 = i0;
		size_t need = 0;
		while (i1 < n_jobs) {
			const int ql = pos ? pos[i1].qlen : jobs[i1].qlen, tl = pos ? pos[i1].tlen : jobs[i1].tlen, w = pos ? pos[i1].w : jobs[i1].w;
			size_t t = 128;
			if (ql > 0 && tl > 0) t = ((size_t)ql + tl) * ((size_t)wm_ksw_ncol(ql, tl, w) + 10) + 512;
			if (i1 > i0 && need + t > budget) break;
			need += t; ++i1;
		}
		wm_ksw_dev_batch_t *b = 0;
		const double ta = now_ms();
		int rc = ksw_prepare_impl(c, sc, i1 - i0, pos ? 0 : jobs + i0, seqs, seqs_bytes, pos ? pos + i0 : 0, &b);
		if (rc) return rc;
		const double tb_ = now_ms();
		rc = wm_ksw_dev_run(c, b);
		const double tc = now_ms();
		size_t u = 0;
		if (!rc) rc = wm_ksw_dev_fetch(c, b, results + i0, cigar_pool + used, cigar_cap - used, &u);
		if (!rc && zd) rc = ksw_fetch_zd(c, b, zd + i0);
		c->acc_cells += b->cells; c->t_prep += tb_ - ta; c->t_run += tc - tb_; c->t_fetch += now_ms() - tc; kms += b->dp_ms + b->bt_ms;
		wm_ksw_dev_free(c, b);
		if (rc) { if (cigar_used) *cigar_used = used + u; return rc; }
		for (int i = i0; i < i1; ++i) results[i].cig_off += (uint32_t)used;
		used += u;
		i0 = i1;
		if (n_jobs == 0) break;
	}
	if (cigar_used) *cigar_used = used;
	c->last_ms = kms;
	return WM_OK;
}

extern "C" int wm_ksw_batch(wm_ctx_t *c, const wm_ksw_score_t *sc, int n_jobs, const wm_ksw_job_t *jobs, const uint8_t *seqs, size_t seqs_bytes,
                            wm_ksw_result_t *results, uint32_t *cigar_pool, size_t cigar_cap, size_t *cigar_used)
{
	return ksw_batch_impl(c, sc, n_jobs, jobs, seqs, seqs_bytes, 0, results, cigar_pool, cigar_cap, cigar_used);
}

extern "C" int wm_ksw_batch_pos(wm_ctx_t *c, const wm_ksw_score_t *sc, int n_jobs, const wm_ksw_pos_t *jobs,
                                wm_ksw_result_t *results, uint32_t *cigar_pool, size_t cigar_cap, size_t *cigar_used)
{
	if (n_jobs > 0 && !jobs) return set_err(WM_EINVAL, "null jobs");
	return ksw_batch_impl(c, sc, n_jobs, 0, 0, 0, jobs, results, cigar_pool, cigar_cap, cigar_used);
}

extern "C" int wm_ksw_batch_pos_zd(wm_ctx_t *c, const wm_ksw_score_t *sc, int n_jobs, const wm_ksw_pos_t *jobs,
                                   wm_ksw_result_t *results, uint32_t *cigar_pool, size_t cigar_cap, size_t *cigar_used, wm_zd_t *zd)
{
	if (n_jobs > 0 && (!jobs || !zd)) return set_err(WM_EINVAL, "null jobs / zd");
	return ksw_batch_impl(c, sc, n_jobs, 0, 0, 0, jobs, results, cigar_pool, cigar_cap, cigar_used, zd);
}

extern "C" int wm_debug_stripe_timing(uint64_t *out16, int reset)
{
#ifdef WM_STRIPE_TIMING
	unsigned long long h[16];
	if (hipMemcpyFromSymbol(h, HIP_SYMBOL(g_wm_stripe_timing), sizeof(h)) != hipSuccess) return set_err(WM_EINTERNAL, "hipMemcpyFromSymbol: %s", hipGetErrorString(hipGetLastError()));
	for (int i = 0; i < 16; ++i) out16[i] = h[i];
	if (reset) { memset(h, 0, sizeof(h)); if (hipMemcpyToSymbol(HIP_SYMBOL(g_wm_stripe_timing), h, sizeof(h)) != hipSuccess) return set_err(WM_EINTERNAL, "hipMemcpyToSymbol failed"); }
	return WM_OK;
#else
	(void)out16; (void)reset;
	return set_err(WM_EINVAL, "this library was not built with WM_STRIPE_TIMING");
#endif
}

extern "C" int wm_ksw_extd2(wm_ctx_t *c, int qlen, const uint8_t *query, int tlen, const uint8_t *target, int8_t m, const int8_t *mat,
                            int8_t q, int8_t e, int8_t q2, int8_t e2, int w, int zdrop, int end_bonus, int flag, wm_ksw_result_t *ez, uint32_t **cigar_out)
{
	if (m != 5) return set_err(WM_EINVAL, "only the 5-letter alphabet of src/align.c:9 is supported");
	wm_ksw_score_t sc = { mat[0], mat[1], mat[24], q, e, q2, e2 };
	wm_ksw_job_t jb = { 0, (uint32_t)(qlen > 0 ? qlen : 0), qlen, tlen, w, zdrop, end_bonus, flag };
	std::vector<uint8_t> seqs((qlen > 0 ? qlen : 0) + (tlen > 0 ? tlen : 0) + 1);
	if (qlen > 0) memcpy(seqs.data(), query, qlen);
	if (tlen > 0) memcpy(seqs.data() + (qlen > 0 ? qlen : 0), target, tlen);
	const size_t cap = (size_t)(qlen > 0 ? qlen : 0) + (tlen > 0 ? tlen : 0) + 4;
	uint32_t *cig = (uint32_t*)malloc(cap * 4);
	size_t used = 0;
	int rc = wm_ksw_batch(c, &sc, 1, &jb, seqs.data(), seqs.size(), ez, cig, cap, &used);
	if (rc) { free(cig); *cigar_out = 0; return rc; }
	*cigar_out = cig;
	return WM_OK;
}

__global__ __launch_bounds__(64) void ksw_exts2_kernel(wm_ksw_score_t sc, int noncan, int junc_bonus, const wm_ksw_djob_t *__restrict__ jobs,
                                                        const uint8_t *__restrict__ seqs, const uint8_t *__restrict__ junc, uint8_t *__restrict__ tb,
                                                        uint8_t *scratch, const uint64_t *__restrict__ scratch_off, wm_ksw_dres_t *__restrict__ res)
{
	const int j = blockIdx.x;
	const wm_ksw_djob_t jb = jobs[j];
	const uint64_t T = ((uint64_t)jb.tlen + 15) / 16 * 16;
	signed char *mem = (signed char*)(scratch + scratch_off[j]);
	wmk::ksw_dp_exts2<true>(sc, noncan, junc_bonus, jb, seqs, junc, tb, mem, (int*)(mem + 8 * T), res + j);
}
__global__ __launch_bounds__(64) void ksw_exts2_backtrack_kernel(wm_ksw_score_t sc, int n, const wm_ksw_djob_t *__restrict__ jobs, const uint8_t *__restrict__ tb,
                                                                  wm_ksw_dres_t *__restrict__ res, uint32_t *__restrict__ cig_scratch, int *__restrict__ err)
{
	const int j = blockIdx.x * 64 + threadIdx.x;
	if (j >= n) return;
	wm_ksw_dres_t r = res[j];
	int nc = 0;
	if (r.bt_i == KSW_BT_WATCHDOG) atomicMax(err, 2);
	if (r.bt_i >= 0) {
		nc = wmk::ksw_exts2_backtrack_thread(sc, jobs[j], tb, r.bt_i, r.bt_j, cig_scratch + jobs[j].cig_off, jobs[j].cig_cap);
		if (nc < 0) { atomicMax(err, 1); nc = 0; }
	}
	res[j].n_cigar = nc;
}

extern "C" int wm_ksw_exts2_batch(wm_ctx_t *c, const wm_ksw_score_t *sc_in, int noncan, int junc_bonus, int n_jobs, const wm_ksw_job_t *jobs,
                                  const uint8_t *seqs, size_t seqs_bytes, const uint8_t *junc,
                                  wm_ksw_result_t *results, uint32_t *cigar_pool, size_t cigar_cap, size_t *cigar_used)
try {
	if (!c) return set_err(WM_EINVAL, "null context");
	if (cigar_used) *cigar_used = 0;
	if (n_jobs < 0) return set_err(WM_EINVAL, "n_jobs < 0");
	if (n_jobs == 0) return WM_OK;
	if (!sc_in || !jobs || !seqs || !results) return set_err(WM_EINVAL, "null argument");
	const wm_ksw_score_t sc = *sc_in;
	if (sc.e <= 0 || sc.q2 <= sc.q + sc.e) return set_err(WM_EINVAL, "ksw_exts2 needs e > 0 and q2 > q + e (src/ksw2_exts2_sse.c:66)");
	if (-(int)sc.mismatch > 2 * (sc.q + sc.e)) return set_err(WM_EINVAL, "mismatch penalty above 2 (q + e): the reference returns without aligning (src/ksw2_exts2_sse.c:84)");
	if (noncan < -127 || noncan > 127 || junc_bonus < -127 || junc_bonus > 127) return set_err(WM_EINVAL, "noncan / junc_bonus are int8 in the reference");
	HIPCHK(hipSetDevice(c->device));
	ArenaMark mark(c);
	std::vector<wm_ksw_djob_t> dj(n_jobs);
	std::vector<uint64_t> soff(n_jobs);
	uint64_t tb_off = 0, cig_off = 0, sc_off = 0;
	for (int i = 0; i < n_jobs; ++i) {
		const wm_ksw_job_t &jb = jobs[i];
		if (jb.qlen <= 0 || jb.tlen <= 0) return set_err(WM_EINVAL, "job %d: empty operand", i);
		if ((uint64_t)jb.q_off + jb.qlen > seqs_bytes || (uint64_t)jb.t_off + jb.tlen > seqs_bytes) return set_err(WM_EINVAL, "job %d: operands outside seqs", i);
		if (jb.flag & (0x01 | 0x04 | 0x10)) return set_err(WM_EINVAL, "job %d: KSW_EZ_SCORE_ONLY / GENERIC_SC / APPROX_DROP are not supported", i);
		wm_ksw_djob_t &d = dj[i];
		memset(&d, 0, sizeof(d));
		d.q_off = jb.q_off; d.t_off = jb.t_off; d.qlen = jb.qlen; d.tlen = jb.tlen; d.w = -1; d.zdrop = jb.zdrop; d.end_bonus = 0; d.flag = jb.flag;
		d.n_col = (((jb.qlen < jb.tlen ? jb.qlen : jb.tlen) + 15) / 16 + 1) * 16;
		d.tb_off = tb_off;
		tb_off += ((uint64_t)(jb.qlen + jb.tlen - 1) * d.n_col + 15) & ~(uint64_t)15;
		d.cig_off = (uint32_t)cig_off; d.cig_cap = jb.qlen + jb.tlen + 2;
		cig_off += d.cig_cap;
		soff[i] = sc_off;
		sc_off += (12 * (((uint64_t)jb.tlen + 15) / 16 * 16) + 256 + 255) & ~(uint64_t)255;
	}
	if (cig_off >= ((uint64_t)1 << 32)) return set_err(WM_ENOMEM, "ksw_exts2: batch too large (split it)");
	const size_t nj = (size_t)n_jobs;
	wm_ksw_djob_t *d_jobs = (wm_ksw_djob_t*)arena_take(c, nj * sizeof(wm_ksw_djob_t));
	uint64_t *d_soff = (uint64_t*)arena_take(c, nj * 8);
	wm_ksw_dres_t *d_res = (wm_ksw_dres_t*)arena_take(c, nj * sizeof(wm_ksw_dres_t));
	uint32_t *d_off = (uint32_t*)arena_take(c, nj * 4 + 64);
	uint32_t *d_total = (uint32_t*)arena_take(c, 64);
	int *d_err = (int*)arena_take(c, 64);
	uint8_t *d_seqs = (uint8_t*)arena_take(c, seqs_bytes + 64);
	uint8_t *d_junc = junc ? (uint8_t*)arena_take(c, seqs_bytes + 64) : 0;
	uint32_t *d_cig = (uint32_t*)arena_take(c, (cig_off + 16) * 4);
	uint32_t *d_pool = (uint32_t*)arena_take(c, (cig_off + 16) * 4);
	uint8_t *d_scratch = (uint8_t*)arena_take(c, sc_off + 256);
	uint8_t *d_tb = (uint8_t*)arena_take(c, tb_off + 64);
	if (!d_jobs || !d_soff || !d_res || !d_off || !d_total || !d_err || !d_seqs || (junc && !d_junc) || !d_cig || !d_pool || !d_scratch || !d_tb)
		return set_err(WM_ENOMEM, "ksw_exts2: batch does not fit the arena (%llu traceback bytes); split it", (unsigned long long)tb_off);
	HIPCHK(hipMemcpyAsync(d_jobs, dj.data(), nj * sizeof(wm_ksw_djob_t), hipMemcpyHostToDevice, c->stream));
	HIPCHK(hipMemcpyAsync(d_soff, soff.data(), nj * 8, hipMemcpyHostToDevice, c->stream));
	HIPCHK(hipMemcpyAsync(d_seqs, seqs, seqs_bytes, hipMemcpyHostToDevice, c->stream));
	if (junc) HIPCHK(hipMemcpyAsync(d_junc, junc, seqs_bytes, hipMemcpyHostToDevice, c->stream));
	HIPCHK(hipMemsetAsync(d_err, 0, 4, c->stream));
	hipLaunchKernelGGL(ksw_exts2_kernel, dim3(n_jobs), dim3(64), 0, c->stream, sc, noncan, junc_bonus, d_jobs, d_seqs, d_junc, d_tb, d_scratch, d_soff, d_res);
	hipLaunchKernelGGL(ksw_exts2_backtrack_kernel, dim3((n_jobs + 63) / 64), dim3(64), 0, c->stream, sc, n_jobs, d_jobs, d_tb, d_res, d_cig, d_err);
	hipLaunchKernelGGL(ksw_scan_kernel, dim3(1), dim3(1024), 0, c->stream, n_jobs, d_res, d_off, d_total);
	hipLaunchKernelGGL(ksw_gather_kernel, dim3(n_jobs), dim3(64), 0, c->stream, d_jobs, d_res, d_off, d_cig, d_pool, (uint32_t)(cig_off + 16));
	HIPCHK(hipGetLastError());
	UBuf<wm_ksw_dres_t> res(nj, c);
	UBuf<uint32_t> off(nj, c);
	UBuf<uint32_t> small(4, c);
	HIPCHK(hipMemcpyAsync(res.data(), d_res, nj * sizeof(wm_ksw_dres_t), hipMemcpyDeviceToHost, c->stream));
	HIPCHK(hipMemcpyAsync(off.data(), d_off, nj * 4, hipMemcpyDeviceToHost, c->stream));
	HIPCHK(hipMemcpyAsync(small.data(), d_total, 4, hipMemcpyDeviceToHost, c->stream));
	HIPCHK(hipMemcpyAsync(small.data() + 1, d_err, 4, hipMemcpyDeviceToHost, c->stream));
	HIPCHK(ctx_sync(c));
	if (small[1]) return set_err(WM_EINTERNAL, "cigar slot overflow in backtrack");
	const uint32_t total = small[0];
	if (cigar_used) *cigar_used = total;
	if (total > cigar_cap) return set_err(WM_ENOMEM, "cigar_pool too small: need %u ops", total);
	if (total) {
		if (!cigar_pool) return set_err(WM_EINVAL, "null cigar_pool");
		HIPCHK(hipMemcpyAsync(cigar_pool, d_pool, (size_t)total * 4, hipMemcpyDeviceToHost, c->stream));
		HIPCHK(ctx_sync(c));
	}
	for (int i = 0; i < n_jobs; ++i) {
		wm_ksw_result_t &o = results[i];
		const wm_ksw_dres_t &r = res[i];
		o.max = r.max; o.zdropped = r.zdropped; o.max_q = r.max_q; o.max_t = r.max_t; o.mqe = r.mqe; o.mqe_t = r.mqe_t;
		o.mte = r.mte; o.mte_q = r.mte_q; o.score = r.score; o.reach_end = r.reach_end; o.n_cigar = r.n_cigar; o.cig_off = off[i];
	}
	return WM_OK;
}
catch (const std::bad_alloc &) { return set_err(WM_ENOMEM, "out of host memory"); }
```

### winnowmap_amd/gpu.py

```python
import ctypes as C
import os
import numpy as np

HERE = os.path.dirname(os.path.abspath(__file__))
LIB_PATH = os.environ.get("WM_LIBWMGPU") or os.path.join(HERE, "libwmgpu.so")


class WmError(RuntimeError):
    pass


class KswScore(C.Structure):
    _fields_ = [("match", C.c_int8), ("mismatch", C.c_int8), ("sc_ambi", C.c_int8),
                ("q", C.c_int8), ("e", C.c_int8), ("q2", C.c_int8), ("e2", C.c_int8)]


KSW_JOB_DTYPE = np.dtype([("q_off", np.uint32), ("t_off", np.uint32), ("qlen", np.int32), ("tlen", np.int32),
                          ("w", np.int32), ("zdrop", np.int32), ("end_bonus", np.int32), ("flag", np.int32)])
KSW_RES_DTYPE = np.dtype([("max", np.int32), ("zdropped", np.int32), ("max_q", np.int32), ("max_t", np.int32),
                          ("mqe", np.int32), ("mqe_t", np.int32), ("mte", np.int32), ("mte_q", np.int32),
                          ("score", np.int32), ("reach_end", np.int32), ("n_cigar", np.int32), ("cig_off", np.uint32)])

KSW_F_ZDWALK = 0x10000
KSW_POS_DTYPE = np.dtype([("qwin_off", np.int64), ("qwin_len", np.int32), ("q_pos", np.int32), ("rid", np.int32), ("t_pos", np.int32),
                          ("qlen", np.int32), ("tlen", np.int32), ("w", np.int32), ("zdrop", np.int32), ("end_bonus", np.int32), ("flag", np.int32),
                          ("step", np.int8), ("has_n", np.int8), ("pad", np.int8, (6,))])

_lib = None


def lib():
    global _lib
    if _lib is None:
        if not os.path.exists(LIB_PATH):
            raise WmError("libwmgpu.so is not built (run `python -m winnowmap_amd.build`); there is no CPU fallback")
        L = C.CDLL(LIB_PATH)
        L.wm_last_error.restype = C.c_char_p
        L.wm_ctx_create.argtypes = [C.c_int, C.c_size_t, C.POINTER(C.c_void_p)]
        L.wm_ctx_destroy.argtypes = [C.c_void_p]
        L.wm_last_kernel_ms.restype = C.c_float
        L.wm_last_kernel_ms.argtypes = [C.c_void_p]
        L.wm_ksw_batch.argtypes = [C.c_void_p, C.POINTER(KswScore), C.c_int, C.c_void_p, C.c_void_p, C.c_size_t,
                                   C.c_void_p, C.c_void_p, C.c_size_t, C.POINTER(C.c_size_t)]
        L.wm_ksw_dev_prepare.argtypes = [C.c_void_p, C.POINTER(KswScore), C.c_int, C.c_void_p, C.c_void_p, C.c_size_t, C.POINTER(C.c_void_p)]
        L.wm_ksw_dev_run.argtypes = [C.c_void_p, C.c_void_p]
        L.wm_ksw_dev_fetch.argtypes = [C.c_void_p, C.c_void_p, C.c_void_p, C.c_void_p, C.c_size_t, C.POINTER(C.c_size_t)]
        L.wm_ksw_dev_stats.argtypes = [C.c_void_p, C.POINTER(C.c_uint64), C.POINTER(C.c_uint64), C.POINTER(C.c_float), C.POINTER(C.c_float)]
        L.wm_ksw_dev_free.argtypes = [C.c_void_p, C.c_void_p]
        _lib = L
    return _lib


def _chk(rc):
    if rc != 0:
        raise WmError("libwmgpu error %d: %s" % (rc, lib().wm_last_error().decode()))


class Context:

    def __init__(self, device=0, arena_bytes=0):
        self._h = C.c_void_p()
        _chk(lib().wm_ctx_create(device, arena_bytes, C.byref(self._h)))

    def close(self):
        if self._h:
            lib().wm_ctx_destroy(self._h)
            self._h = C.c_void_p()

    def __del__(self):
        try:
            self.close()
        except Exception:
            pass

    def ksw_batch(self, score, jobs, seqs):
        jobs = np.ascontiguousarray(jobs, KSW_JOB_DTYPE)
        seqs = np.ascontiguousarray(seqs, np.uint8)
        res = np.zeros(len(jobs), KSW_RES_DTYPE)
        cap = int((jobs["qlen"].astype(np.int64) + jobs["tlen"] + 2).sum()) + 16
        pool = np.zeros(cap, np.uint32)
        used = C.c_size_t(0)
        _chk(lib().wm_ksw_batch(self._h, C.byref(score), len(jobs), jobs.ctypes.data, seqs.ctypes.data, seqs.nbytes,
                                res.ctypes.data, pool.ctypes.data, cap, C.byref(used)))
        return res, pool[:used.value]

    def ksw_exts2_batch(self, score, noncan, junc_bonus, jobs, seqs, junc=None):
        jobs = np.ascontiguousarray(jobs, KSW_JOB_DTYPE)
        seqs = np.ascontiguousarray(seqs, np.uint8)
        jn = None if junc is None else np.ascontiguousarray(junc, np.uint8)
        assert jn is None or jn.nbytes == seqs.nbytes
        res = np.zeros(len(jobs), KSW_RES_DTYPE)
        cap = int((jobs["qlen"].astype(np.int64) + jobs["tlen"] + 2).sum()) + 16
        pool = np.zeros(cap, np.uint32)
        used = C.c_size_t(0)
        lib().wm_ksw_exts2_batch.argtypes = [C.c_void_p, C.POINTER(KswScore), C.c_int, C.c_int, C.c_int, C.c_void_p, C.c_void_p, C.c_size_t, C.c_void_p,
                                             C.c_void_p, C.c_void_p, C.c_size_t, C.POINTER(C.c_size_t)]
        _chk(lib().wm_ksw_exts2_batch(self._h, C.byref(score), noncan, junc_bonus, len(jobs), jobs.ctypes.data, seqs.ctypes.data, seqs.nbytes,
                                      None if jn is None else jn.ctypes.data, res.ctypes.data, pool.ctypes.data, cap, C.byref(used)))
        return res, pool[:used.value]

    def reads_upload(self, codes):
        codes = np.ascontiguousarray(codes, np.uint8)
        lib().wm_reads_upload.argtypes = [C.c_void_p, C.c_void_p, C.c_size_t]
        _chk(lib().wm_reads_upload(self._h, codes.ctypes.data, codes.nbytes))

    def ksw_batch_pos(self, score, jobs):
        jobs = np.ascontiguousarray(jobs, KSW_POS_DTYPE)
        assert KSW_POS_DTYPE.itemsize == 56
        res = np.zeros(len(jobs), KSW_RES_DTYPE)
        cap = int((np.maximum(jobs["qlen"], 0).astype(np.int64) + np.maximum(jobs["tlen"], 0) + 2).sum()) + 16
        pool = np.zeros(cap, np.uint32)
        used = C.c_size_t(0)
        lib().wm_ksw_batch_pos.argtypes = [C.c_void_p, C.POINTER(KswScore), C.c_int, C.c_void_p, C.c_void_p, C.c_void_p, C.c_size_t, C.POINTER(C.c_size_t)]
        _chk(lib().wm_ksw_batch_pos(self._h, C.byref(score), len(jobs), jobs.ctypes.data, res.ctypes.data, pool.ctypes.data, cap, C.byref(used)))
        return res, pool[:used.value]

    def ksw_batch_pos_zd(self, score, jobs):
        jobs = np.ascontiguousarray(jobs, KSW_POS_DTYPE)
        res = np.zeros(len(jobs), KSW_RES_DTYPE)
        cap = int((np.maximum(jobs["qlen"], 0).astype(np.int64) + np.maximum(jobs["tlen"], 0) + 2).sum()) + 16
        pool = np.zeros(cap, np.uint32)
        zd = np.zeros((len(jobs), 5), np.int32)
        used = C.c_size_t(0)
        lib().wm_ksw_batch_pos_zd.argtypes = [C.c_void_p, C.POINTER(KswScore), C.c_int, C.c_void_p, C.c_void_p, C.c_void_p, C.c_size_t, C.POINTER(C.c_size_t), C.c_void_p]
        _chk(lib().wm_ksw_batch_pos_zd(self._h, C.byref(score), len(jobs), jobs.ctypes.data, res.ctypes.data, pool.ctypes.data, cap, C.byref(used), zd.ctypes.data))
        return res, pool[:used.value], zd

    def seed_batch_keyed(self, mini, mini_off, n_mini, qlen, keys, max_occ, flag, out_cap):
        L = lib()
        L.wm_seed_batch_keyed.argtypes = [C.c_void_p, C.c_int] + [C.c_void_p] * 5 + [C.c_int, C.c_int64, C.c_void_p, C.c_size_t] + [C.c_void_p] * 3
        n = len(n_mini)
        mini = np.ascontiguousarray(mini, np.uint64)
        mini_off, n_mini, qlen = np.ascontiguousarray(mini_off, np.uint64), np.ascontiguousarray(n_mini, np.int32), np.ascontiguousarray(qlen, np.int32)
        keys = None if keys is None else np.ascontiguousarray(keys, np.uint32).reshape(n, 2)
        out = np.zeros((out_cap, 2), np.uint64)
        out_off, n_a, rep_len = np.zeros(n, np.uint64), np.zeros(n, np.int32), np.zeros(n, np.int32)
        _chk(L.wm_seed_batch_keyed(self._h, n, mini.ctypes.data, mini_off.ctypes.data, n_mini.ctypes.data, qlen.ctypes.data, None if keys is None else keys.ctypes.data,
                                   max_occ, flag, out.ctypes.data, out_cap, out_off.ctypes.data, n_a.ctypes.data, rep_len.ctypes.data))
        return out, out_off, n_a, rep_len

    def window_batch_keyed(self, jobs, keys, seqs, pre, max_occ, flag, u_cap, a_cap):
        L = lib()
        L.wm_window_batch_keyed.argtypes = [C.c_void_p, C.c_int, C.c_void_p, C.c_void_p, C.c_void_p, C.c_size_t, C.c_void_p, C.c_size_t, C.c_int, C.c_int64,
                                            C.c_void_p, C.c_void_p, C.c_size_t, C.c_void_p, C.c_void_p, C.c_size_t, C.c_void_p]
        n = len(jobs)
        jobs = np.ascontiguousarray(jobs, WINDOW_JOB)
        keys = None if keys is None else np.ascontiguousarray(keys, np.uint32).reshape(n, 2)
        seqs = np.ascontiguousarray(seqs, np.uint8)
        pre = np.ascontiguousarray(pre, np.uint64).reshape(-1, 2)
        res = np.zeros(n, WINDOW_RES)
        u_pool, a_pool = np.zeros(u_cap + 1, np.uint64), np.zeros((a_cap + 1, 2), np.uint64)
        uu, au = C.c_size_t(), C.c_size_t()
        _chk(L.wm_window_batch_keyed(self._h, n, jobs.ctypes.data, None if keys is None else keys.ctypes.data, seqs.ctypes.data, seqs.nbytes, pre.ctypes.data, len(pre),
                                     max_occ, flag, res.ctypes.data, u_pool.ctypes.data, u_cap, C.byref(uu), a_pool.ctypes.data, a_cap, C.byref(au)))
        return res, u_pool[:uu.value], a_pool[:au.value]

    def ksw_prepare(self, score, jobs, seqs):
        jobs = np.ascontiguousarray(jobs, KSW_JOB_DTYPE)
        seqs = np.ascontiguousarray(seqs, np.uint8)
        h = C.c_void_p()
        _chk(lib().wm_ksw_dev_prepare(self._h, C.byref(score), len(jobs), jobs.ctypes.data, seqs.ctypes.data, seqs.nbytes, C.byref(h)))
        return KswDevBatch(self, h, jobs)


class KswDevBatch:
    def __init__(self, ctx, h, jobs):
        self.ctx, self._h, self.jobs = ctx, h, jobs

    def run(self):
        _chk(lib().wm_ksw_dev_run(self.ctx._h, self._h))

    def stats(self):
        cells, tbb, dp, bt = C.c_uint64(), C.c_uint64(), C.c_float(), C.c_float()
        lib().wm_ksw_dev_stats(self._h, C.byref(cells), C.byref(tbb), C.byref(dp), C.byref(bt))
        return dict(cells=cells.value, tb_bytes=tbb.value, dp_ms=dp.value, bt_ms=bt.value)

    def fetch(self):
        res = np.zeros(len(self.jobs), KSW_RES_DTYPE)
        cap = int((self.jobs["qlen"].astype(np.int64) + self.jobs["tlen"] + 2).sum()) + 16
        pool = np.zeros(cap, np.uint32)
        used = C.c_size_t(0)
        _chk(lib().wm_ksw_dev_fetch(self.ctx._h, self._h, res.ctypes.data, pool.ctypes.data, cap, C.byref(used)))
        return res, pool[:used.value]

    def free(self):
        if self._h:
            lib().wm_ksw_dev_free(self.ctx._h, self._h)
            self._h = None


def set_ksw_routing(on=-1, rows4=-1, rows8=-1):
    lib().wm_ksw_set_routing.argtypes = [C.c_int, C.c_int, C.c_int]
    lib().wm_ksw_set_routing.restype = None
    lib().wm_ksw_set_routing(on, rows4, rows8)


def set_ksw_chain_routing(mode=-1, min_rows_exact=-1, bp=-1):
    lib().wm_ksw_set_chain_routing.argtypes = [C.c_int, C.c_int, C.c_int]
    lib().wm_ksw_set_chain_routing.restype = None
    lib().wm_ksw_set_chain_routing(mode, min_rows_exact, bp)


def set_ksw_dual(on):
    lib().wm_ksw_set_dual.argtypes = [C.c_int]
    lib().wm_ksw_set_dual.restype = None
    lib().wm_ksw_set_dual(int(on))


def ksw_dual_enabled():
    lib().wm_ksw_dual_enabled.restype = C.c_int
    return bool(lib().wm_ksw_dual_enabled())


def build_defines():
    lib().wm_build_defines.restype = C.c_char_p
    return lib().wm_build_defines().decode()


STRIPE_TIMING_FIELDS = ("scan", "epoch", "cells", "wait_left", "book", "wait_right", "publish", "rows", "epochs", "total", "waves")


def stripe_timing(reset=True):
    out = np.zeros(16, np.uint64)
    lib().wm_debug_stripe_timing.argtypes = [C.c_void_p, C.c_int]
    _chk(lib().wm_debug_stripe_timing(out.ctypes.data, 1 if reset else 0))
    return {k: int(out[i]) for i, k in enumerate(STRIPE_TIMING_FIELDS)}


def pack_jobs(pairs, w=751, zdrop=400, end_bonus=-1, flag=0):
    jobs = np.zeros(len(pairs), KSW_JOB_DTYPE)
    chunks, off = [], 0
    for i, p in enumerate(pairs):
        q, t = np.asarray(p[0], np.uint8), np.asarray(p[1], np.uint8)
        o = dict(w=w, zdrop=zdrop, end_bonus=end_bonus, flag=flag)
        if len(p) > 2:
            o.update(p[2])
        jobs[i] = (off, off + len(q), len(q), len(t), o["w"], o["zdrop"], o["end_bonus"], o["flag"])
        chunks += [q, t]
        off += len(q) + len(t)
    seqs = np.concatenate(chunks) if chunks else np.zeros(0, np.uint8)
    return jobs, seqs


WINDOW_JOB = np.dtype([("seq_off", "<i8"), ("stage_off", "<u8"), ("pre_off", "<u8"), ("len", "<i4"), ("n_pre", "<i4"),
                       ("max_dist_x", "<i4"), ("min_dist_x", "<i4"), ("max_dist_y", "<i4"), ("bw", "<i4"), ("max_skip", "<i4"), ("max_iter", "<i4"), ("min_cnt", "<i4"), ("min_sc", "<i4"),
                       ("gap_scale", "<f4"), ("is_cdna", "<i4")])
WINDOW_RES = np.dtype([("n_anchors", "<i4"), ("rep_len", "<i4"), ("n_mini", "<i4"), ("n_u", "<i4"), ("n_v", "<i4"), ("u_off", "<u4"), ("a_off", "<u4")])


def _bind_map(L):
    if getattr(L, "_wm_map_bound", False):
        return
    L.wm_index_build.argtypes = [C.c_char_p, C.c_char_p, C.c_int, C.c_int, C.c_int, C.POINTER(C.c_void_p)]
    L.wm_index_destroy.argtypes = [C.c_void_p]
    L.wm_index_upload.argtypes = [C.c_void_p, C.c_void_p]
    L.wm_index_n_seq.argtypes = [C.c_void_p]
    L.wm_index_seq_name.restype = C.c_char_p
    L.wm_index_seq_name.argtypes = [C.c_void_p, C.c_int]
    L.wm_index_seq_len.argtypes = [C.c_void_p, C.c_int]
    L.wm_index_n_minimizers.restype = C.c_uint64
    L.wm_index_n_minimizers.argtypes = [C.c_void_p]
    L.wm_mapper_create.argtypes = [C.c_void_p, C.c_void_p, C.c_char_p, C.c_int64, C.POINTER(C.c_void_p)]
    L.wm_mapper_destroy.argtypes = [C.c_void_p]
    L.wm_mapper_set_threads.argtypes = [C.c_void_p, C.c_int, C.c_size_t]
    L.wm_map_reads.argtypes = [C.c_void_p, C.c_int, C.POINTER(C.c_char_p), C.POINTER(C.c_char_p), C.c_void_p,
                               C.POINTER(C.c_char_p), C.POINTER(C.c_size_t), C.POINTER(C.c_void_p), C.POINTER(C.c_void_p), C.POINTER(C.c_void_p)]
    L.wm_map_reads_slot.argtypes = [C.c_void_p, C.c_int] + list(L.wm_map_reads.argtypes[1:])
    L.wm_mapper_stats.argtypes = [C.c_void_p, C.c_void_p]
    L.wm_sam_header.argtypes = [C.c_void_p, C.c_int, C.POINTER(C.c_char_p), C.POINTER(C.c_char_p), C.POINTER(C.c_size_t)]
    L.wm_last_aux_ms.restype = C.c_float
    L.wm_last_aux_ms.argtypes = [C.c_void_p]
    L.wm_write_repetitive_kmers.argtypes = [C.c_char_p, C.c_int, C.c_double, C.c_char_p, C.POINTER(C.c_uint64)]
    L.wm_index_export.argtypes = [C.c_void_p] + [C.c_void_p] * 8
    L.wm_index_import.argtypes = [C.c_void_p] * 8 + [C.POINTER(C.c_void_p)]
    L._wm_map_bound = True


def write_repetitive_kmers(fasta, k, out_path, distinct=0.9998):
    L = lib()
    _bind_map(L)
    n = C.c_uint64()
    _chk(L.wm_write_repetitive_kmers(os.fsencode(fasta), k, distinct, os.fsencode(out_path), C.byref(n)))
    return int(n.value)


def write_repetitive_kmers_gpu(ctx, fasta, k, out_path, distinct=0.9998):
    L = lib()
    L.wm_write_repetitive_kmers_gpu.argtypes = [C.c_void_p, C.c_char_p, C.c_int, C.c_double, C.c_char_p, C.POINTER(C.c_uint64), C.c_void_p]
    n = C.c_uint64()
    st = np.zeros(4, np.float64)
    _chk(L.wm_write_repetitive_kmers_gpu(ctx._h, os.fsencode(fasta), k, distinct, os.fsencode(out_path), C.byref(n), st.ctypes.data))
    return int(n.value), {"read_encode_s": float(st[0]), "device_s": float(st[1]), "write_s": float(st[2]), "distinct_kmers": int(st[3])}


_EXPORT_DTYPES = (np.uint32, np.uint64, np.uint64, np.uint64, np.uint8, np.uint64, np.uint8)


class MapOpt(C.Structure):
    _fields_ = [("flag", C.c_int64)] + [(n, C.c_int32) for n in ("seed", "sdust_thres", "max_qlen", "bw", "max_gap", "max_gap_ref", "min_gap_ref", "max_frag_len",
                                                                  "max_chain_skip", "max_chain_iter", "min_cnt", "min_chain_score")] + \
               [("chain_gap_scale", C.c_float)] + [(n, C.c_int32) for n in ("SVaware", "SVawareMinReadLength", "suffixSampleOffset", "min_mapq")] + [("min_qcov", C.c_float)] + \
               [(n, C.c_int32) for n in ("minPrefixLength", "maxPrefixLength")] + [("prefixIncrementFactor", C.c_float)] + \
               [(n, C.c_int32) for n in ("stage2_bw", "stage2_zdrop_inv", "stage2_max_gap")] + [("mask_level", C.c_float), ("mask_len", C.c_int32), ("pri_ratio", C.c_float), ("best_n", C.c_int32)] + \
               [(n, C.c_int32) for n in ("max_join_long", "max_join_short", "min_join_flank_sc")] + [("min_join_flank_ratio", C.c_float), ("alt_drop", C.c_float)] + \
               [(n, C.c_int32) for n in ("a", "b", "q", "e", "q2", "e2", "sc_ambi", "zdrop", "zdrop_inv", "end_bonus", "min_dp_max", "min_ksw_len")] + \
               [("max_clip_ratio", C.c_float), ("mid_occ_frac", C.c_float)] + [(n, C.c_int32) for n in ("min_mid_occ", "mid_occ", "max_occ")] + [("mini_batch_size", C.c_int64), ("max_sw_mat", C.c_int64)] + \
               [(n, C.c_int32) for n in ("noncan", "junc_bonus", "anchor_ext_len", "anchor_ext_shift")]


def mapopt_preset(preset):
    L = lib()
    L.wm_mapopt_preset.argtypes = [C.c_char_p, C.POINTER(MapOpt), C.POINTER(C.c_int), C.POINTER(C.c_int)]
    o = MapOpt(); k = C.c_int(); w = C.c_int()
    _chk(L.wm_mapopt_preset((preset or "").encode(), C.byref(o), C.byref(k), C.byref(w)))
    return o, k.value, w.value


def build_index_parts(fasta, kmer_file, k, w, batch_bases, n_threads=8):
    L = lib()
    _bind_map(L)
    L.wm_index_build_parts.argtypes = [C.c_char_p, C.c_char_p, C.c_int, C.c_int, C.c_int, C.c_uint64, C.POINTER(C.c_void_p), C.c_int, C.POINTER(C.c_int)]
    cap = 4096
    arr = (C.c_void_p * cap)()
    n = C.c_int()
    _chk(L.wm_index_build_parts(os.fsencode(fasta), os.fsencode(kmer_file) if kmer_file else None, k, w, n_threads, batch_bases, arr, cap, C.byref(n)))
    return [Index(_handle=C.c_void_p(arr[i])) for i in range(n.value)]


def map_file_multi(mappers, reads_path, out_path, mini_batch_bases=0):
    L = lib()
    L.wm_map_file_multi.argtypes = [C.POINTER(C.c_void_p), C.c_int, C.c_char_p, C.c_char_p, C.c_int64, C.c_void_p]
    arr = (C.c_void_p * len(mappers))(*[m._h for m in mappers])
    st = np.zeros(6, np.float64)
    _chk(L.wm_map_file_multi(arr, len(mappers), os.fsencode(reads_path), os.fsencode(out_path), mini_batch_bases, st.ctypes.data))
    return dict(zip(("reads", "bases", "batches", "t_read", "t_map", "t_write"), (float(x) for x in st)))


def map_file_split(ctx, parts, opt, n_threads, reads_path, out_path, mini_batch_bases=0):
    L = lib()
    L.wm_map_file_split.argtypes = [C.c_void_p, C.c_int, C.POINTER(C.c_void_p), C.POINTER(MapOpt), C.c_int, C.c_char_p, C.c_char_p, C.c_int64, C.c_void_p]
    arr = (C.c_void_p * len(parts))(*[p._h for p in parts])
    st = np.zeros(6, np.float64)
    _chk(L.wm_map_file_split(ctx._h, len(parts), arr, C.byref(opt), n_threads, os.fsencode(reads_path), os.fsencode(out_path), mini_batch_bases, st.ctypes.data))
    return dict(zip(("reads", "bases", "batches", "t_read", "t_map", "t_write"), (float(x) for x in st)))


def map_file_split_fasta(ctx, fasta, kmer_file, k, w, batch_bases, opt, n_threads, reads_path, out_path, on_device=False, build_threads=8, mini_batch_bases=0):
    L = lib()
    L.wm_map_file_split_fasta.argtypes = [C.c_void_p, C.c_char_p, C.c_char_p, C.c_int, C.c_int, C.c_int, C.c_uint64, C.c_int, C.POINTER(MapOpt), C.c_int,
                                          C.c_char_p, C.c_char_p, C.c_int64, C.c_void_p, C.POINTER(C.c_int)]
    st = np.zeros(6, np.float64)
    n = C.c_int()
    _chk(L.wm_map_file_split_fasta(ctx._h, os.fsencode(fasta), os.fsencode(kmer_file) if kmer_file else None, k, w, build_threads, batch_bases, 1 if on_device else 0,
                                   C.byref(opt), n_threads, os.fsencode(reads_path), os.fsencode(out_path), mini_batch_bases, st.ctypes.data, C.byref(n)))
    d = dict(zip(("reads", "bases", "batches", "t_read", "t_map", "t_write"), (float(x) for x in st)))
    d["parts"] = n.value
    return d


class SplitRun:

    def __init__(self, ctx, opt, k, w, n_threads, reads_path, mini_batch_bases=0):
        L = lib()
        L.wm_split_begin.argtypes = [C.c_void_p, C.POINTER(MapOpt), C.c_int, C.c_int, C.c_int, C.c_char_p, C.c_int64, C.POINTER(C.c_void_p)]
        L.wm_split_add_part.argtypes = [C.c_void_p, C.c_void_p]
        L.wm_split_finish.argtypes = [C.c_void_p, C.c_char_p, C.c_void_p]
        L.wm_split_abort.argtypes = [C.c_void_p]
        L.wm_split_abort.restype = None
        self._h = C.c_void_p()
        _chk(L.wm_split_begin(ctx._h, C.byref(opt), k, w, n_threads, os.fsencode(reads_path), mini_batch_bases, C.byref(self._h)))

    def add_part(self, idx):
        _chk(lib().wm_split_add_part(self._h, idx._h))

    def finish(self, out_path):
        st = np.zeros(6, np.float64)
        h, self._h = self._h, None
        _chk(lib().wm_split_finish(h, os.fsencode(out_path), st.ctypes.data))
        return dict(zip(("reads", "bases", "batches", "t_read", "t_map", "t_write"), (float(x) for x in st)))

    def abort(self):
        if self._h:
            lib().wm_split_abort(self._h)
            self._h = None


class Index:

    def __init__(self, fasta=None, kmer_file=None, k=15, w=50, n_threads=8, _handle=None, hpc=False):
        L = lib()
        _bind_map(L)
        self._h = C.c_void_p()
        if _handle is not None:
            self._h = _handle
            return
        L.wm_index_build_flag.argtypes = [C.c_char_p, C.c_char_p, C.c_int, C.c_int, C.c_int, C.c_int, C.POINTER(C.c_void_p)]
        _chk(L.wm_index_build_flag(os.fsencode(fasta), os.fsencode(kmer_file) if kmer_file else None, k, w, 1 if hpc else 0, n_threads, C.byref(self._h)))

    @staticmethod
    def build_on_device(ctx, fasta, kmer_file=None, k=15, w=50, n_threads=8, hpc=False):
        L = lib()
        _bind_map(L)
        L.wm_index_build_gpu_flag.argtypes = [C.c_void_p, C.c_char_p, C.c_char_p, C.c_int, C.c_int, C.c_int, C.c_int, C.POINTER(C.c_void_p), C.c_void_p]
        h = C.c_void_p()
        st = np.zeros(4, np.float64)
        _chk(L.wm_index_build_gpu_flag(ctx._h, os.fsencode(fasta), os.fsencode(kmer_file) if kmer_file else None, k, w, 1 if hpc else 0, n_threads, C.byref(h), st.ctypes.data))
        L.wm_last_aux_ms.restype = C.c_float
        L.wm_last_aux_ms.argtypes = [C.c_void_p]
        return Index(_handle=h), {"read_pack_s": float(st[0]), "device_sketch_s": float(st[1]), "table_s": float(st[2]), "minimizers": int(st[3]),
                                  "table_on_device_s": float(L.wm_last_aux_ms(ctx._h)) * 1e-3}

    def read_junc_bed(self, path):
        L = lib()
        L.wm_index_read_junc_bed.argtypes = [C.c_void_p, C.c_char_p]
        _chk(L.wm_index_read_junc_bed(self._h, os.fsencode(path)))

    def export_arrays(self):
        L = lib()
        sizes = np.zeros(9, np.uint64)
        _chk(L.wm_index_export(self._h, sizes.ctypes.data, None, None, None, None, None, None, None))
        n = [int(sizes[0]), int(sizes[1]), int(sizes[1]), int(sizes[2]), int(sizes[3]), 2 * int(sizes[4]), int(sizes[5])]
        arrs = [np.zeros(max(m, 1), dt) for m, dt in zip(n, _EXPORT_DTYPES)]
        _chk(L.wm_index_export(self._h, sizes.ctypes.data, *[a.ctypes.data for a in arrs]))
        return sizes, arrs

    @staticmethod
    def from_arrays(sizes, arrs):
        L = lib()
        _bind_map(L)
        h = C.c_void_p()
        arrs = [np.ascontiguousarray(a, dt) for a, dt in zip(arrs, _EXPORT_DTYPES)]
        sizes = np.ascontiguousarray(sizes, np.uint64)
        _chk(L.wm_index_import(sizes.ctypes.data, *[a.ctypes.data for a in arrs], C.byref(h)))
        return Index(_handle=h)

    def save(self, path):
        L = lib()
        L.wm_index_save.argtypes = [C.c_void_p, C.c_char_p]
        _chk(L.wm_index_save(self._h, path.encode()))

    @staticmethod
    def load(path, kmer_file=None):
        L = lib()
        _bind_map(L)
        L.wm_index_load.argtypes = [C.c_char_p, C.c_char_p, C.POINTER(C.c_void_p)]
        h = C.c_void_p()
        _chk(L.wm_index_load(path.encode(), kmer_file.encode() if kmer_file else None, C.byref(h)))
        return Index(_handle=h)

    def upload(self, ctx):
        _chk(lib().wm_index_upload(ctx._h, self._h))

    def upload_dev(self, ctx, d_ptrs, src_device):
        L = lib()
        L.wm_index_upload_dev.argtypes = [C.c_void_p, C.c_void_p] + [C.c_void_p] * 5 + [C.c_int]
        _chk(L.wm_index_upload_dev(ctx._h, self._h, *[C.c_void_p(int(p)) for p in d_ptrs], int(src_device)))

    def upload_peer(self, dst_ctx, src_ctx):
        L = lib()
        L.wm_index_upload_peer.argtypes = [C.c_void_p, C.c_void_p, C.c_void_p]
        _chk(L.wm_index_upload_peer(dst_ctx._h, self._h, src_ctx._h))

    @property
    def n_minimizers(self):
        if not self._h:
            raise RuntimeError("the index has been closed")
        return int(lib().wm_index_n_minimizers(self._h))

    def names(self):
        L = lib()
        return [L.wm_index_seq_name(self._h, i).decode() for i in range(L.wm_index_n_seq(self._h))]

    def query_key(self, name):
        return tuple(int(x) for x in self.query_keys([name])[0])

    def query_keys(self, names):
        L = lib()
        L.wm_index_query_key.argtypes = [C.c_void_p, C.c_char_p, C.c_void_p]
        out = np.zeros((len(names), 2), np.uint32)
        for i, nm in enumerate(names):
            _chk(L.wm_index_query_key(self._h, nm if isinstance(nm, bytes) else nm.encode(), out[i:].ctypes.data))
        return out

    def close(self):
        if self._h:
            lib().wm_index_destroy(self._h)
            self._h = C.c_void_p()


MM_F_CIGAR, MM_F_OUT_SAM, MM_F_OUT_CG = 0x4, 0x8, 0x20
MM_F_NO_DIAG, MM_F_NO_DUAL, MM_F_NO_LJOIN, MM_F_ALL_CHAINS = 0x1, 0x2, 0x400, 0x800000
MM_F_AVA = MM_F_ALL_CHAINS | MM_F_NO_DIAG | MM_F_NO_DUAL | MM_F_NO_LJOIN
STAT_NAMES = ("super_steps", "ksw_jobs", "chain_jobs", "seed_jobs", "sketch_jobs", "dp_cells", "ksw_kernel_us", "aux_kernel_us", "read_bases")


class Mapper:

    def __init__(self, ctx, index, preset="map-ont", flag=MM_F_CIGAR | MM_F_OUT_CG):
        L = lib()
        _bind_map(L)
        self.ctx, self.index = ctx, index
        self._h = C.c_void_p()
        _chk(L.wm_mapper_create(ctx._h, index._h, preset.encode() if preset else None, flag, C.byref(self._h)))

    def set_threads(self, n_threads, arena_bytes_per_thread=0):
        _chk(lib().wm_mapper_set_threads(self._h, n_threads, arena_bytes_per_thread))

    @staticmethod
    def marshal(names, seqs):
        n = len(seqs)
        nm = (C.c_char_p * n)(*[x if isinstance(x, bytes) else x.encode() for x in names])
        sq = (C.c_char_p * n)(*seqs)
        lens = np.array([len(s) for s in seqs], np.int32)
        return n, nm, sq, lens, (names, seqs)

    def map(self, names, seqs=None, copy_text=True, slot=0):
        L = lib()
        n, nm, sq, lens, _keep = names if seqs is None else Mapper.marshal(names, seqs)
        text, tlen = C.c_char_p(), C.c_size_t()
        hits, cig, first = C.c_void_p(), C.c_void_p(), C.c_void_p()
        _chk(L.wm_map_reads_slot(self._h, slot, n, nm, sq, lens.ctypes.data, C.byref(text), C.byref(tlen), C.byref(hits), C.byref(cig), C.byref(first)))
        fa = np.ctypeslib.as_array(C.cast(first, C.POINTER(C.c_int64)), shape=(n + 1,)).copy()
        nh = int(fa[n])
        ha = np.ctypeslib.as_array(C.cast(hits, C.POINTER(C.c_int32)), shape=(nh, 16)).copy() if nh else np.zeros((0, 16), np.int32)
        if not copy_text:
            return tlen.value, ha, None, fa
        nc = int(ha[:, 7].sum()) if nh else 0
        ca = np.ctypeslib.as_array(C.cast(cig, C.POINTER(C.c_uint32)), shape=(nc,)).copy() if nc else np.zeros(0, np.uint32)
        return C.string_at(text, tlen.value), ha, ca, fa

    def rep_len_defined(self, slot=0):
        L = lib()
        L.wm_map_reads_rep_len_defined.argtypes = [C.c_void_p, C.c_int, C.POINTER(C.c_void_p), C.POINTER(C.c_size_t)]
        p, n = C.c_void_p(), C.c_size_t()
        _chk(L.wm_map_reads_rep_len_defined(self._h, slot, C.byref(p), C.byref(n)))
        return np.ctypeslib.as_array(C.cast(p, C.POINTER(C.c_uint8)), shape=(n.value,)).copy() if n.value else np.zeros(0, np.uint8)

    def stats(self):
        a = np.zeros(9, np.uint64)
        lib().wm_mapper_stats(self._h, a.ctypes.data)
        return dict(zip(STAT_NAMES, (int(x) for x in a)))

    def map_file(self, reads_path, out_path, mini_batch_bases=0):
        L = lib()
        L.wm_map_file.argtypes = [C.c_void_p, C.c_char_p, C.c_char_p, C.c_int64, C.c_void_p]
        st = np.zeros(6, np.float64)
        _chk(L.wm_map_file(self._h, reads_path.encode(), out_path.encode(), mini_batch_bases, st.ctypes.data))
        return dict(zip(("reads", "bases", "batches", "t_read", "t_map", "t_write"), (float(x) for x in st)))

    def kernel_stats(self):
        out = np.zeros(3 * 64, np.float64)
        n = C.c_int()
        lib().wm_mapper_kernel_stats.argtypes = [C.c_void_p, C.c_void_p, C.c_int, C.POINTER(C.c_int)]
        _chk(lib().wm_mapper_kernel_stats(self._h, out.ctypes.data, len(out), C.byref(n)))
        return {k: (float(out[3 * k]), float(out[3 * k + 1]), int(out[3 * k + 2])) for k in range(n.value)}

    def kernel_union(self, since_ms=0.0):
        ncl = int(lib().wm_ksw_n_classes())
        out = np.zeros(max(64, ncl), np.float64)
        now = C.c_double()
        lib().wm_mapper_kernel_union.argtypes = [C.c_void_p, C.c_double, C.c_void_p, C.c_int, C.POINTER(C.c_double)]
        _chk(lib().wm_mapper_kernel_union(self._h, float(since_ms), out.ctypes.data, len(out), C.byref(now)))
        return {k: float(out[k]) for k in range(ncl)}, now.value

    def host_stats(self):
        a = np.zeros(24, np.float64)
        lib().wm_mapper_host_stats.argtypes = [C.c_void_p, C.c_void_p, C.c_int]
        _chk(lib().wm_mapper_host_stats(self._h, a.ctypes.data, len(a)))
        ops = ("window", "seed", "chain", "ksw")
        return {"cpu_glue_s": float(a[0]), "idle_wall_s": float(a[1]), "cpu_batched_s": {o: float(a[2 + i]) for i, o in enumerate(ops)},
                "wall_batched_s": {o: float(a[6 + i]) for i, o in enumerate(ops)}, "batched_calls": {o: int(a[10 + i]) for i, o in enumerate(ops)},
                "map_wall_s": float(a[14]), "format_wall_s": float(a[15]), "threads": int(a[16]), "cpu_help_s": float(a[17]),
                "glue_wall_s": float(a[18]), "lock_wait_wall_s": float(a[19]), "workers_wall_s": float(a[20])}

    def close(self):
        if self._h:
            lib().wm_mapper_destroy(self._h)
            self._h = C.c_void_p()
```

Before: 0.1664.

## Parallelize cigar offset scan, split backtrack by job length, pin result readback

Replaces the single-block serial prefix scan over cigar counts with a two-pass wave-level scan over a compact ncig array. The gather reads counts from that array and skips empty jobs. Backtrack can route long jobs to a cooperative wave kernel through a sorted order list; by default every job uses the thread kernel. Results and z-drop data are copied back into persistent pinned host buffers, so fetch no longer needs its own staging allocations and extra syncs. This adds kernel launches and host-side bookkeeping, and it changes the arena budget to include chain mailbox bytes.

```diff
diff --git a/__graft_entry__.py b/__graft_entry__.py
--- a/__graft_entry__.py
+++ b/__graft_entry__.py
@@ -12,6 +12,7 @@
     b.build_oracle()
     b.build_emu()
     b.build_emu_selfmap()
+    b.build_emu_tail()
     b.build_emu_chain()
     b.build_harness()
     import winnowmap_amd
diff --git a/include/wm_gpu.h b/include/wm_gpu.h
--- a/include/wm_gpu.h
+++ b/include/wm_gpu.h
@@ -80,6 +80,7 @@
 
 void wm_ksw_set_routing(int on, int rows4, int rows8);
 void wm_ksw_set_chain_routing(int mode, int min_rows_exact, int bp);
+void wm_ksw_set_bt_walk(int mode);
 void wm_ksw_set_dual(int on);
 int wm_ksw_dual_enabled(void);
 
diff --git a/winnowmap_amd/build.py b/winnowmap_amd/build.py
--- a/winnowmap_amd/build.py
+++ b/winnowmap_amd/build.py
@@ -116,6 +116,17 @@
     return out
 
 
+def build_emu_tail():
+    emu = os.path.join(ROOT, "tests", "simt_emu")
+    out = os.path.join(emu, "libwm_emu_tail.so")
+    srcs = [os.path.join(emu, f) for f in ("emu_tail.cpp", "simt.h")] + [os.path.join(CSRC, "ksw_tail.h")]
+    with _Lock(out):
+        if _newer(out, srcs):
+            _run_to(out, lambda o: ["g++", "-O1", "-std=c++17", "-fPIC", "-shared", "-ffp-contract=off", "-Wno-unknown-pragmas",
+                                    "-I" + emu, "-I" + CSRC, "-o", o, os.path.join(emu, "emu_tail.cpp")])
+    return out
+
+
 def build_emu_stripe(defines=()):
     emu = os.path.join(ROOT, "tests", "simt_emu")
     tag = "".join("_" + "".join(ch if ch.isalnum() else "_" for ch in d) for d in defines)
@@ -159,6 +170,7 @@
     build_oracle()
     build_emu()
     build_emu_selfmap()
+    build_emu_tail()
     build_emu_stripe()
     build_emu_chain()
     build_harness()
diff --git a/winnowmap_amd/csrc/ksw_tail.h b/winnowmap_amd/csrc/ksw_tail.h
--- /dev/null
+++ b/winnowmap_amd/csrc/ksw_tail.h
@@ -0,0 +1,45 @@
+#pragma once
+#include <stdint.h>
+
+#define KSW_SCAN_K 4
+#define KSW_SCAN_CHUNK (64 * KSW_SCAN_K)
+
+namespace wmk {
+using namespace simt;
+
+WM_DEV int ksw_scan_sum(const uint32_t *__restrict__ a, int b, int e)
+{
+	const V<int> ln = lane();
+	V<int> s = 0;
+	for (int i = b; i < e; i += 64) {
+		const V<int> idx = ln + i;
+		WM_IF(idx < e) s = wadd(s, cast<int>(gld(a, idx))); WM_END
+	}
+	return readlane(wave_scan_add(s), 63);
+}
+
+WM_DEV void ksw_scan_partial(int g, int n, const uint32_t *__restrict__ nc, uint32_t *__restrict__ wsum)
+{
+	const int b = g * KSW_SCAN_CHUNK, e = b + KSW_SCAN_CHUNK < n ? b + KSW_SCAN_CHUNK : n;
+	const int s = ksw_scan_sum(nc, b, e);
+	WM_IF(lane() == 0) gst(wsum, (long long)g, (uint32_t)s); WM_END
+}
+
+WM_DEV void ksw_scan_offsets(int g, int n, const uint32_t *__restrict__ nc, const uint32_t *__restrict__ wsum,
+                             uint32_t *__restrict__ off, uint32_t *__restrict__ total)
+{
+	const V<int> ln = lane();
+	const int b = g * KSW_SCAN_CHUNK;
+	int carry = ksw_scan_sum(wsum, 0, g);
+	for (int k = 0; k < KSW_SCAN_K; ++k) {
+		const V<int> idx = ln + (b + 64 * k);
+		V<int> v = 0;
+		WM_IF(idx < n) v = cast<int>(gld(nc, idx)); WM_END
+		const V<int> inc = wave_scan_add(v);
+		WM_IF(idx < n) gst(off, idx, cast<uint32_t>(wadd(wsub(inc, v), carry))); WM_END
+		carry = wadd(carry, readlane(inc, 63));
+	}
+	if (b + KSW_SCAN_CHUNK >= n) { WM_IF(ln == 0) gst(total, 0ll, (uint32_t)carry); WM_END }
+}
+
+}
diff --git a/winnowmap_amd/csrc/wm_ksw.hip b/winnowmap_amd/csrc/wm_ksw.hip
--- a/winnowmap_amd/csrc/wm_ksw.hip
+++ b/winnowmap_amd/csrc/wm_ksw.hip
@@ -8,6 +8,7 @@
 #include "ksw_chain_kernel.h"
 #include "ksw_exts2_kernel.h"
 #include "cigar_walk.h"
+#include "ksw_tail.h"
 #include "reads2bit.h"
 
 #ifndef WM_OCC_HINT
@@ -116,13 +117,14 @@
 	wmk::ksw_dp_chain<BP, CLIP, HASN, EXACT>(sc, jb, seqs, tb, mb, (int)m.w, (int)m.y, tbs, res + j);
 }
 
-__global__ __launch_bounds__(256) void ksw_reset_kernel(int n, const wm_ksw_djob_t *__restrict__ jobs, wm_ksw_dres_t *__restrict__ res)
+__global__ __launch_bounds__(256) void ksw_reset_kernel(int n, const wm_ksw_djob_t *__restrict__ jobs, wm_ksw_dres_t *__restrict__ res, uint32_t *__restrict__ ncig)
 {
 	const int j = blockIdx.x * 256 + threadIdx.x;
 	if (j >= n || jobs[j].klass >= 0) return;
 	wm_ksw_dres_t z;
 	z.max = 0; z.zdropped = 0; z.max_q = z.max_t = z.mqe_t = z.mte_q = -1; z.score = z.mqe = z.mte = KSW_NEG_INF; z.reach_end = 0; z.n_cigar = 0; z.bt_i = z.bt_j = -1;
 	res[j] = z;
+	ncig[j] = 0;
 }
 
 __global__ __launch_bounds__(64) void ksw_expand_kernel(const wm_ksw_djob_t *__restrict__ jobs, const wm_ksw_dsrc_t *__restrict__ src,
@@ -149,28 +151,31 @@
 	}
 }
 
-__global__ __launch_bounds__(64) void ksw_backtrack_kernel(int n, const wm_ksw_djob_t *__restrict__ jobs, const uint8_t *__restrict__ tb,
-                                                            wm_ksw_dres_t *__restrict__ res, uint32_t *__restrict__ cig_scratch, int *__restrict__ err)
+__global__ __launch_bounds__(64) void ksw_backtrack_kernel(int n, const int *__restrict__ order, int wave_rows, const wm_ksw_djob_t *__restrict__ jobs, const uint8_t *__restrict__ tb,
+                                                            wm_ksw_dres_t *__restrict__ res, uint32_t *__restrict__ ncig, uint32_t *__restrict__ cig_scratch, int *__restrict__ err)
 {
 	WM_SETPRIO(3);
-	const int j = blockIdx.x * 64 + threadIdx.x;
-	if (j >= n) return;
-	wm_ksw_dres_t r = res[j];
+	const int i = blockIdx.x * 64 + threadIdx.x;
+	if (i >= n) return;
+	const int j = order[i];
+	if (jobs[j].qlen + jobs[j].tlen >= wave_rows) return;
+	const int bt_i = res[j].bt_i, bt_j = res[j].bt_j;
 	int nc = 0;
-	if (r.bt_i == KSW_BT_WATCHDOG) atomicMax(err, 2);
-	if (r.bt_i >= 0) {
-		nc = wmk::ksw_backtrack_thread(jobs[j], tb, r.bt_i, r.bt_j, cig_scratch + jobs[j].cig_off, jobs[j].cig_cap);
+	if (bt_i == KSW_BT_WATCHDOG) atomicMax(err, 2);
+	if (bt_i >= 0) {
+		nc = wmk::ksw_backtrack_thread(jobs[j], tb, bt_i, bt_j, cig_scratch + jobs[j].cig_off, jobs[j].cig_cap);
 		if (nc < 0) { atomicMax(err, 1); nc = 0; }
 	}
 	res[j].n_cigar = nc;
-}
-
-__global__ __launch_bounds__(64) void ksw_backtrack_coop_kernel(int n, const wm_ksw_djob_t *__restrict__ jobs, const uint8_t *__restrict__ tb,
-                                                                 wm_ksw_dres_t *__restrict__ res, uint32_t *__restrict__ cig_scratch, int *__restrict__ err)
+	ncig[j] = (uint32_t)nc;
+}
+
+__global__ __launch_bounds__(64) void ksw_backtrack_coop_kernel(const int *__restrict__ order, const wm_ksw_djob_t *__restrict__ jobs, const uint8_t *__restrict__ tb,
+                                                                 wm_ksw_dres_t *__restrict__ res, uint32_t *__restrict__ ncig, uint32_t *__restrict__ cig_scratch, int *__restrict__ err)
 {
 	WM_SETPRIO(3);
 	__shared__ uint8_t tile[KSW_BT_ROWS * 64];
-	const int j = blockIdx.x;
+	const int j = order[blockIdx.x];
 	const int bt_i = res[j].bt_i, bt_j = res[j].bt_j;
 	int nc = 0;
 	if (bt_i == KSW_BT_WATCHDOG && threadIdx.x == 0) atomicMax(err, 2);
@@ -178,38 +183,43 @@
 		nc = wmk::ksw_backtrack_wave(jobs[j], tb, bt_i, bt_j, cig_scratch + jobs[j].cig_off, jobs[j].cig_cap, tile);
 		if (nc < 0) { if (threadIdx.x == 0) atomicMax(err, 1); nc = 0; }
 	}
-	if (threadIdx.x == 0) res[j].n_cigar = nc;
-}
-
-__global__ __launch_bounds__(1024) void ksw_scan_kernel(int n, const wm_ksw_dres_t *__restrict__ res, uint32_t *__restrict__ off, uint32_t *__restrict__ total)
+	if (threadIdx.x == 0) { res[j].n_cigar = nc; ncig[j] = (uint32_t)nc; }
+}
+
+__global__ __launch_bounds__(256) void ksw_scan_partial_kernel(int n, const uint32_t *__restrict__ ncig, uint32_t *__restrict__ wsum)
 {
 	WM_SETPRIO(3);
-	__shared__ uint32_t part[1024];
-	const int tid = threadIdx.x, per = (n + 1023) / 1024, b = tid * per, e = b + per < n ? b + per : n;
-	uint32_t s = 0;
-	for (int i = b; i < e; ++i) s += (uint32_t)res[i].n_cigar;
-	part[tid] = s;
-	__syncthreads();
-	if (tid == 0) {
-		uint32_t acc = 0;
-		for (int i = 0; i < 1024; ++i) { uint32_t t = part[i]; part[i] = acc; acc += t; }
-		*total = acc;
-	}
-	__syncthreads();
-	s = part[tid];
-	for (int i = b; i < e; ++i) { off[i] = s; s += (uint32_t)res[i].n_cigar; }
-}
-
-__global__ __launch_bounds__(64) void ksw_gather_kernel(const wm_ksw_djob_t *__restrict__ jobs, const wm_ksw_dres_t *__restrict__ res,
+	const int g = (int)blockIdx.x * 4 + simt::wave_in_block();
+	if ((long long)g * KSW_SCAN_CHUNK >= n) return;
+	wmk::ksw_scan_partial(g, n, ncig, wsum);
+}
+__global__ __launch_bounds__(256) void ksw_scan_offsets_kernel(int n, const uint32_t *__restrict__ ncig, const uint32_t *__restrict__ wsum, uint32_t *__restrict__ off, uint32_t *__restrict__ total)
+{
+	WM_SETPRIO(3);
+	const int g = (int)blockIdx.x * 4 + simt::wave_in_block();
+	if ((long long)g * KSW_SCAN_CHUNK >= n) return;
+	wmk::ksw_scan_offsets(g, n, ncig, wsum, off, total);
+}
+static inline int ksw_scan_waves(int n) { return (n + KSW_SCAN_CHUNK - 1) / KSW_SCAN_CHUNK; }
+static void ksw_scan_launch(hipStream_t s, int n, const uint32_t *ncig, uint32_t *wsum, uint32_t *off, uint32_t *total)
+{
+	const int nb = (ksw_scan_waves(n) + 3) / 4;
+	hipLaunchKernelGGL(ksw_scan_partial_kernel, dim3(nb), dim3(256), 0, s, n, ncig, wsum);
+	hipLaunchKernelGGL(ksw_scan_offsets_kernel, dim3(nb), dim3(256), 0, s, n, ncig, wsum, off, total);
+}
+
+__global__ __launch_bounds__(64) void ksw_gather_kernel(const wm_ksw_djob_t *__restrict__ jobs, const uint32_t *__restrict__ ncig,
                                                          const uint32_t *__restrict__ off, const uint32_t *__restrict__ cig_scratch,
                                                          uint32_t *__restrict__ pool, uint32_t pool_cap)
 {
 	WM_SETPRIO(3);
-	const int j = blockIdx.x, n = res[j].n_cigar;
+	const int j = blockIdx.x, n = (int)ncig[j];
+	if (n == 0) return;
 	const uint32_t *src = cig_scratch + jobs[j].cig_off;
 	const bool rev = (jobs[j].flag & KSW_F_REV_CIGAR) != 0;
+	const uint32_t o = off[j];
 	for (int i = threadIdx.x; i < n; i += 64) {
-		const uint32_t dst = off[j] + (uint32_t)i;
+		const uint32_t dst = o + (uint32_t)i;
 		if (dst < pool_cap) pool[dst] = src[rev ? i : n - 1 - i];
 	}
 }
@@ -227,6 +237,23 @@
 	zd[j] = z;
 }
 
+struct PinBlock {
+	uint8_t *p = 0; size_t mark = 0; bool pinned = false;
+	bool take(wm_ctx_t *c, size_t bytes)
+	{
+		p = (uint8_t*)pin_take(c, bytes ? bytes : 1, &mark);
+		pinned = p != 0;
+		if (!p) p = (uint8_t*)malloc(bytes ? bytes : 1);
+		return p != 0;
+	}
+	void release(wm_ctx_t *c)
+	{
+		if (pinned) { if (c && c->pin_used >= mark) pin_release(c, mark); }
+		else free(p);
+		p = 0; pinned = false;
+	}
+};
+
 struct wm_ksw_dev_batch_s {
 	int n_jobs;
 	wm_ksw_score_t sc, sc_in;
@@ -234,12 +261,19 @@
 	std::vector<wm_ksw_djob_t> jobs;
 	std::vector<int> order[WM_KSW_NCLASS];
 	std::vector<int> ord;
+	std::vector<int> ord_long;
+	int long_off[WM_KSW_NCLASS + 1];
+	int wave_rows;
 	std::vector<int> degenerate;
 	std::vector<std::string> dumped;
 	uint8_t *d_gscratch; uint64_t *d_goff; std::vector<uint64_t> goff;
 	uint8_t *d_b3state; uint64_t *d_b3off; std::vector<uint64_t> b3off;
 	std::vector<uint4> cmap[WM_KSW_NCLASS - WM_KSW_CHAIN][2]; uint4 *d_cmap[WM_KSW_NCLASS - WM_KSW_CHAIN][2]; wm_mbox_t *d_mail = 0; size_t mail_words = 0; int *d_tickets = 0;
-	wm_ksw_djob_t *d_jobs; int *d_order; uint8_t *d_seqs, *d_tb; wm_ksw_dres_t *d_res; uint32_t *d_cig, *d_off, *d_total, *d_pool; int *d_err;
+	wm_ksw_djob_t *d_jobs; int *d_order, *d_order_long; uint8_t *d_seqs, *d_tb; wm_ksw_dres_t *d_res; uint32_t *d_cig, *d_off, *d_total, *d_pool, *d_nc, *d_wsum; int *d_err;
+	size_t back_bytes, o_off, o_zd, o_err;
+	PinBlock tab, back;
+	wm_ctx_t *ctx = 0;
+	~wm_ksw_dev_batch_s() { back.release(ctx); tab.release(ctx); }
 	size_t pool_cap, arena_mark, slab_bytes;
 	uint64_t cells, tb_bytes;
 	uint64_t class_cells[WM_KSW_NCLASS];
@@ -337,6 +371,34 @@
 	if (bp == 2 || bp == 4) g_chain_geom = bp == 4 ? 1 : 0;
 }
 
+#ifndef WM_KSW_BT_WAVE_ROWS_DEFAULT
+#define WM_KSW_BT_WAVE_ROWS_DEFAULT INT_MAX
+#endif
+static std::atomic<int> g_bt_wave_rows(-1);
+static int bt_rows_of_mode(int mode) { return mode == 0 ? INT_MAX : mode == 1 ? 0 : mode >= 2 ? mode : WM_KSW_BT_WAVE_ROWS_DEFAULT; }
+static int bt_wave_rows()
+{
+	int v = g_bt_wave_rows.load(std::memory_order_relaxed);
+	if (v < 0) {
+		const char *e = getenv("WM_KSW_COOP_BT"), *r = getenv("WM_KSW_BT_WAVE_ROWS");
+		v = e && *e ? bt_rows_of_mode(atoi(e) > 0 ? 1 : 0) : r && atoi(r) >= 2 ? atoi(r) : WM_KSW_BT_WAVE_ROWS_DEFAULT;
+		g_bt_wave_rows = v;
+	}
+	return v;
+}
+extern "C" void wm_ksw_set_bt_walk(int mode) { g_bt_wave_rows = mode < 0 ? -1 : bt_rows_of_mode(mode); }
+
+static size_t chain_mail_bytes(int qlen, int tlen, int w, int flag)
+{
+	int n_col = 0;
+	int k = wm_ksw_classify(qlen, tlen, w, 0, flag, &n_col);
+	if (stripe_min_rows(0)) k = wm_ksw_route(k, n_col, qlen, tlen, w, 0, stripe_min_rows(4), stripe_min_rows(8), g_stripe_wide16.load(std::memory_order_relaxed));
+	k = wm_ksw_route_chain(k, qlen, tlen, w, 0, flag, chain_mode(), g_chain_rows.load(std::memory_order_relaxed), g_chain_geom.load(std::memory_order_relaxed));
+	if (k < WM_KSW_CHAIN) return 0;
+	const int nwv = wm_chain_nwv(n_col, tlen, 128 * wm_ksw_chain_bp[(k - WM_KSW_CHAIN) >> 2]);
+	return (((size_t)wm_chain_box::words(nwv) + 15) & ~(size_t)15) * 8;
+}
+
 static int ksw_prepare_impl(wm_ctx_t *c, const wm_ksw_score_t *sc_in, int n_jobs, const wm_ksw_job_t *jobs, const uint8_t *seqs, size_t seqs_bytes,
                             const wm_ksw_pos_t *pos, wm_ksw_dev_batch_t **out)
 {
@@ -350,11 +412,12 @@
 	if (pos && !c->d_reads) return set_err(WM_EINVAL, "position jobs need wm_reads_upload on this context");
 	HIPCHK(hipSetDevice(c->device));
 	wm_ksw_dev_batch_t *b = new wm_ksw_dev_batch_t();
+	b->ctx = c; b->wave_rows = bt_wave_rows();
 	b->n_jobs = n_jobs; b->sc = sc; b->sc_in = *sc_in; b->cells = b->tb_bytes = 0; b->dp_ms = b->bt_ms = 0; b->total_ops = 0; b->h_err = 0;
 	memset(b->class_cells, 0, sizeof(b->class_cells));
 	b->arena_mark = c->arena_used;
 	b->jobs.resize(n_jobs);
-	UBuf<wm_ksw_dsrc_t> dsrc(pos ? n_jobs : 0, c);
+	UBuf<wm_ksw_dsrc_t> dsrc(pos ? n_jobs : 0);
 	size_t slab_lo = 0, slab_bytes = 0;
 	int bad0 = -1;
 	if (pos) {
@@ -456,6 +519,11 @@
 			o.swap(tmp);
 		}
 	}
+	b->long_off[0] = 0;
+	for (int k = 0; k < WM_KSW_NCLASS; ++k) {
+		for (int j : b->order[k]) if (b->jobs[j].qlen + b->jobs[j].tlen >= b->wave_rows) b->ord_long.push_back(j);
+		b->long_off[k + 1] = (int)b->ord_long.size();
+	}
 	size_t chain_mw = 0;
 	bool chain_any = false;
 	for (int kc = 0; kc < WM_KSW_NCLASS - WM_KSW_CHAIN; ++kc) {
@@ -473,22 +541,32 @@
 	}
 	const size_t nj = n_jobs > 0 ? n_jobs : 1;
 	auto al256 = [](size_t x) { return (x + 255) & ~(size_t)255; };
-	const size_t o_ord = al256(nj * sizeof(wm_ksw_djob_t)), o_src = o_ord + al256(nj * sizeof(int));
-	size_t o_cm[WM_KSW_NCLASS - WM_KSW_CHAIN][2], tab_bytes = o_src + (pos ? al256(nj * sizeof(wm_ksw_dsrc_t)) : 0);
+	uint64_t go = 0, so = 0;
+	for (int j : b->order[WM_KSW_GENERIC]) { const uint64_t T = ((uint64_t)b->jobs[j].tlen + 15) / 16 * 16; b->goff.push_back(go); go += 12 * T + 256; }
+	for (int j : b->order[WM_KSW_BLOCK3]) { b->b3off.push_back(so); so += 3 * wm_ksw_blk3_wn(b->jobs[j].tlen); }
+	const size_t o_ord = al256(nj * sizeof(wm_ksw_djob_t)), o_lng = o_ord + al256(nj * sizeof(int)), o_src = o_lng + al256(b->ord_long.size() * sizeof(int));
+	const size_t o_goff = o_src + (pos ? al256(nj * sizeof(wm_ksw_dsrc_t)) : 0), o_b3off = o_goff + al256(b->goff.size() * 8);
+	size_t o_cm[WM_KSW_NCLASS - WM_KSW_CHAIN][2], tab_bytes = o_b3off + al256(b->b3off.size() * 8);
 	for (int kc = 0; kc < WM_KSW_NCLASS - WM_KSW_CHAIN; ++kc)
 		for (int e = 0; e < 2; ++e) { o_cm[kc][e] = tab_bytes; tab_bytes += al256(b->cmap[kc][e].size() * sizeof(uint4)); }
 	uint8_t *d_tab = (uint8_t*)arena_take(c, tab_bytes);
 	b->d_jobs = (wm_ksw_djob_t*)d_tab;
 	b->d_order = d_tab ? (int*)(d_tab + o_ord) : 0;
+	b->d_order_long = d_tab ? (int*)(d_tab + o_lng) : 0;
 	for (int kc = 0; kc < WM_KSW_NCLASS - WM_KSW_CHAIN && d_tab; ++kc)
 		for (int e = 0; e < 2; ++e) if (!b->cmap[kc][e].empty()) b->d_cmap[kc][e] = (uint4*)(d_tab + o_cm[kc][e]);
-	b->d_res = (wm_ksw_dres_t*)arena_take(c, al256(nj * sizeof(wm_ksw_dres_t)) + nj * 4 + 64);
-	b->d_off = b->d_res ? (uint32_t*)((uint8_t*)b->d_res + al256(nj * sizeof(wm_ksw_dres_t))) : 0;
-	b->d_err = (int*)arena_take(c, 64);
-	b->d_total = b->d_err ? (uint32_t*)(b->d_err + 1) : 0;
 	bool any_zd = false;
 	for (int i = 0; i < n_jobs && !any_zd; ++i) any_zd = (b->jobs[i].flag & WM_KSW_F_ZDWALK) != 0;
-	b->d_zd = any_zd ? (wm_zd_t*)arena_take(c, nj * sizeof(wm_zd_t)) : 0;
+	b->o_off = al256(nj * sizeof(wm_ksw_dres_t)); b->o_zd = b->o_off + al256(nj * 4); b->o_err = b->o_zd + (any_zd ? al256(nj * sizeof(wm_zd_t)) : 0);
+	b->back_bytes = b->o_err + 64;
+	uint8_t *d_back = (uint8_t*)arena_take(c, b->back_bytes);
+	b->d_res = (wm_ksw_dres_t*)d_back;
+	b->d_off = d_back ? (uint32_t*)(d_back + b->o_off) : 0;
+	b->d_zd = any_zd && d_back ? (wm_zd_t*)(d_back + b->o_zd) : 0;
+	b->d_err = d_back ? (int*)(d_back + b->o_err) : 0;
+	b->d_total = b->d_err ? (uint32_t*)(b->d_err + 1) : 0;
+	b->d_nc = (uint32_t*)arena_take(c, nj * 4 + 64);
+	b->d_wsum = (uint32_t*)arena_take(c, (size_t)ksw_scan_waves((int)nj) * 4 + 64);
 	b->d_seqs = (uint8_t*)arena_take(c, slab_bytes + 64);
 	b->slab_bytes = slab_bytes;
 	wm_ksw_dsrc_t *d_src = pos && d_tab ? (wm_ksw_dsrc_t*)(d_tab + o_src) : 0;
@@ -497,16 +575,11 @@
 	b->d_pool = (uint32_t*)arena_take(c, b->pool_cap * 4);
 	b->d_tb = (uint8_t*)arena_take(c, tb_off + 64);
 	{
-		uint64_t go = 0;
-		for (int j : b->order[WM_KSW_GENERIC]) { const uint64_t T = ((uint64_t)b->jobs[j].tlen + 15) / 16 * 16; b->goff.push_back(go); go += 12 * T + 256; }
 		b->d_gscratch = (uint8_t*)arena_take(c, go + 256);
-		b->d_goff = (uint64_t*)arena_take(c, b->goff.size() * 8 + 64);
-		if (!b->d_gscratch || !b->d_goff) b->d_tb = 0;
-		uint64_t so = 0;
-		for (int j : b->order[WM_KSW_BLOCK3]) { b->b3off.push_back(so); so += 3 * wm_ksw_blk3_wn(b->jobs[j].tlen); }
+		b->d_goff = d_tab ? (uint64_t*)(d_tab + o_goff) : 0;
 		b->d_b3state = (uint8_t*)arena_take(c, so * 4 + 256);
-		b->d_b3off = (uint64_t*)arena_take(c, b->b3off.size() * 8 + 64);
-		if (!b->d_b3state || !b->d_b3off) b->d_tb = 0;
+		b->d_b3off = d_tab ? (uint64_t*)(d_tab + o_b3off) : 0;
+		if (!b->d_gscratch || !b->d_b3state) b->d_tb = 0;
 	}
 	if (chain_any) {
 		b->mail_words = chain_mw;
@@ -514,28 +587,30 @@
 		b->d_tickets = (int*)arena_take(c, 64 * sizeof(int));
 		if (!b->d_mail || !b->d_tickets) b->d_tb = 0;
 	}
-	if (!b->d_jobs || !b->d_order || !b->d_res || !b->d_off || !b->d_total || !b->d_err || !b->d_seqs || (any_zd && !b->d_zd) || (pos && !d_src) || !b->d_cig || !b->d_pool || !b->d_tb) {
+	if (!b->d_jobs || !b->d_order || !b->d_res || !b->d_nc || !b->d_wsum || !b->d_seqs || !b->d_cig || !b->d_pool || !b->d_tb) {
 		c->arena_used = b->arena_mark;
 		delete b;
-		return set_err(WM_ENOMEM, "batch needs %.1f MB of traceback + buffers; arena is %.1f MB", (tb_off + cig_off * 8 + slab_bytes) / 1048576.0, c->arena_bytes / 1048576.0);
-	}
+		return set_err(WM_ENOMEM, "batch needs %.1f MB of traceback + buffers (%.1f MB of them mailboxes: %zu words); arena is %.1f MB",
+		               (tb_off + cig_off * 8 + slab_bytes + chain_mw * 8) / 1048576.0, chain_mw * 8 / 1048576.0, chain_mw, c->arena_bytes / 1048576.0);
+	}
+	if (!b->tab.take(c, tab_bytes) || !b->back.take(c, b->back_bytes)) { c->arena_used = b->arena_mark; delete b; return set_err(WM_ENOMEM, "out of host memory"); }
 	b->ord.clear();
 	b->ord.reserve(nj);
 	for (int k = 0; k < WM_KSW_NCLASS; ++k) b->ord.insert(b->ord.end(), b->order[k].begin(), b->order[k].end());
-	UBuf<uint8_t> ptab(tab_bytes, c);
-	if (n_jobs) memcpy(ptab.data(), b->jobs.data(), (size_t)n_jobs * sizeof(wm_ksw_djob_t));
-	if (!b->ord.empty()) memcpy(ptab.data() + o_ord, b->ord.data(), b->ord.size() * sizeof(int));
-	if (pos && n_jobs > 0) memcpy(ptab.data() + o_src, dsrc.data(), (size_t)n_jobs * sizeof(wm_ksw_dsrc_t));
+	uint8_t *ptab = b->tab.p;
+	if (n_jobs) memcpy(ptab, b->jobs.data(), (size_t)n_jobs * sizeof(wm_ksw_djob_t));
+	if (!b->ord.empty()) memcpy(ptab + o_ord, b->ord.data(), b->ord.size() * sizeof(int));
+	if (!b->ord_long.empty()) memcpy(ptab + o_lng, b->ord_long.data(), b->ord_long.size() * sizeof(int));
+	if (pos && n_jobs > 0) memcpy(ptab + o_src, dsrc.data(), (size_t)n_jobs * sizeof(wm_ksw_dsrc_t));
+	if (!b->goff.empty()) memcpy(ptab + o_goff, b->goff.data(), b->goff.size() * 8);
+	if (!b->b3off.empty()) memcpy(ptab + o_b3off, b->b3off.data(), b->b3off.size() * 8);
 	for (int kc = 0; kc < WM_KSW_NCLASS - WM_KSW_CHAIN; ++kc)
 		for (int e = 0; e < 2; ++e)
-			if (!b->cmap[kc][e].empty()) memcpy(ptab.data() + o_cm[kc][e], b->cmap[kc][e].data(), b->cmap[kc][e].size() * sizeof(uint4));
-	HIPCHK(hipMemcpyAsync(d_tab, ptab.data(), tab_bytes, hipMemcpyHostToDevice, c->stream));
+			if (!b->cmap[kc][e].empty()) memcpy(ptab + o_cm[kc][e], b->cmap[kc][e].data(), b->cmap[kc][e].size() * sizeof(uint4));
+	HIPCHK(hipMemcpyAsync(d_tab, ptab, tab_bytes, hipMemcpyHostToDevice, c->stream));
 	if (pos) {
 		if (n_jobs > 0) hipLaunchKernelGGL(ksw_expand_kernel, dim3(n_jobs), dim3(64), 0, c->stream, b->d_jobs, d_src, c->d_reads, c->d_reads_nm, c->d_S, b->d_seqs);
 	} else if (slab_bytes) HIPCHK(hipMemcpyAsync(b->d_seqs, seqs + slab_lo, slab_bytes, hipMemcpyHostToDevice, c->stream));
-	if (!b->goff.empty()) HIPCHK(hipMemcpyAsync(b->d_goff, b->goff.data(), b->goff.size() * 8, hipMemcpyHostToDevice, c->stream));
-	if (!b->b3off.empty()) HIPCHK(hipMemcpyAsync(b->d_b3off, b->b3off.data(), b->b3off.size() * 8, hipMemcpyHostToDevice, c->stream));
-	HIPCHK(ctx_sync(c));
 	*out = b;
 	return WM_OK;
 }
@@ -543,7 +618,9 @@
 extern "C" int wm_ksw_dev_prepare(wm_ctx_t *c, const wm_ksw_score_t *sc_in, int n_jobs, const wm_ksw_job_t *jobs,
                                   const uint8_t *seqs, size_t seqs_bytes, wm_ksw_dev_batch_t **out)
 {
-	return ksw_prepare_impl(c, sc_in, n_jobs, jobs, seqs, seqs_bytes, 0, out);
+	int rc = ksw_prepare_impl(c, sc_in, n_jobs, jobs, seqs, seqs_bytes, 0, out);
+	if (!rc && hipSuccess != ctx_sync(c)) { wm_ksw_dev_free(c, *out); *out = 0; rc = set_err(WM_ENODEV, "wm_ksw_dev_prepare: the upload failed: %s", hipGetErrorString(hipGetLastError())); }
+	return rc;
 }
 
 int reads_alloc(wm_ctx_t *c, size_t cap)
@@ -589,7 +666,7 @@
 		HIPCHK(hipMemsetAsync(b->d_mail, 0xff, b->mail_words * 8, c->stream));
 		HIPCHK(hipMemsetAsync(b->d_tickets, 0, 64 * sizeof(int), c->stream));
 	}
-	if (!b->degenerate.empty()) hipLaunchKernelGGL(ksw_reset_kernel, dim3((n + 255) / 256), dim3(256), 0, c->stream, n, b->d_jobs, b->d_res);
+	if (!b->degenerate.empty()) hipLaunchKernelGGL(ksw_reset_kernel, dim3((n + 255) / 256), dim3(256), 0, c->stream, n, b->d_jobs, b->d_res, b->d_nc);
 	HIPCHK(hipEventRecord(c->ev[0], c->stream));
 	int off = 0;
 	static const bool trace_k = getenv("WM_TRACE_KSW") != 0;
@@ -644,12 +721,7 @@
 	lorder[nl++] = WM_KSW_GENERIC; lorder[nl++] = WM_KSW_BLOCK3; lorder[nl++] = WM_KSW_BLOCK2; lorder[nl++] = WM_KSW_BLOCK;
 	for (int k = WM_KSW_NCLASS - 1; k >= WM_KSW_STRIPE; --k) lorder[nl++] = k;
 	for (int k = WM_KSW_BLOCK - 1; k >= 0; --k) lorder[nl++] = k;
-	for (int li = 0; li < nl; ++li) {
-		const int k = lorder[li];
-		const int nk = (int)b->order[k].size();
-		if (nk == 0) continue;
-		off = offs[k];
-		next_stream();
+	auto launch_class = [&](const int k, const int nk) -> int {
 		const double tk0 = trace_k ? now_ms() : 0;
 		if (class_events) hipEventRecord(c->cev[k][0], ks);
 		struct Done { decltype(class_done) &f; int k; double t; hipEvent_t e; hipStream_t s; bool on; ~Done() { if (on) hipEventRecord(e, s); f(k, t); } } done_guard{ class_done, k, tk0, c->cev[k][1], ks, class_events };
@@ -671,7 +743,7 @@
 				HIPCHK(hipFuncSetAttribute((const void*)ksw_block_kernel<WM_KSW_BLK2_K, 0>, hipFuncAttributeMaxDynamicSharedMemorySize, (int)lds));
 				hipLaunchKernelGGL((ksw_block_kernel<WM_KSW_BLK2_K, 0>), dim3(nk), dim3(64 * WM_KSW_BLK_NWV), lds, ks, b->sc, b->d_jobs, b->d_order + off, b->d_seqs, b->d_tb, b->d_res, (int)WM_KSW_BLK3_SEQ_LDS, (int*)b->d_b3state, b->d_b3off);
 			}
-			continue;
+			return WM_OK;
 		}
 		if (k >= WM_KSW_CHAIN) {
 			const int kc = k - WM_KSW_CHAIN, var = kc & 3;
@@ -686,7 +758,7 @@
 					else launch_chain<4, false>(var, nw, ks, b->sc, b->d_jobs, b->d_order + off, b->d_seqs, b->d_tb, b->d_res, b->d_cmap[kc][e], b->d_tickets + 2 * kc + e, b->d_mail);
 				}
 			}
-			continue;
+			return WM_OK;
 		}
 		if (k >= WM_KSW_STRIPE) {
 			const int var = (k - WM_KSW_STRIPE) & 3;
@@ -717,11 +789,11 @@
 			case 5: launch_stripe<2, 16>(var, nk, ks, b->sc, b->d_jobs, b->d_order + off, b->d_seqs, b->d_tb, b->d_res); break;
 			default: launch_stripe<8, 8>(var, nk, ks, b->sc, b->d_jobs, b->d_order + off, b->d_seqs, b->d_tb, b->d_res); break;
 			}
-			continue;
+			return WM_OK;
 		}
 		if (k == WM_KSW_GENERIC) {
 			hipLaunchKernelGGL(ksw_generic_kernel, dim3(nk), dim3(64), 0, ks, b->sc, b->d_jobs, b->d_order + off, b->d_seqs, b->d_tb, b->d_gscratch, b->d_goff, b->d_res);
-			continue;
+			return WM_OK;
 		}
 		switch (k & ~7) {
 		case WM_KSW_P4: launch_dpp<4>(k & 7, nk, ks, b->sc, b->d_jobs, b->d_order + off, b->d_seqs, b->d_tb, b->d_res); break;
@@ -746,25 +818,31 @@
 				launch_dpp<16>(k & 7, nk, ks, b->sc, b->d_jobs, b->d_order + off, b->d_seqs, b->d_tb, b->d_res);
 			break;
 		}
+		return WM_OK;
+	};
+	for (int li = 0; li < nl; ++li) {
+		const int k = lorder[li];
+		const int nk = (int)b->order[k].size();
+		if (nk == 0) continue;
+		off = offs[k];
+		next_stream();
+		const int rc_k = launch_class(k, nk);
+		if (rc_k) return rc_k;
+		const int nlong = b->long_off[k + 1] - b->long_off[k];
+		if (nlong > 0) hipLaunchKernelGGL(ksw_backtrack_coop_kernel, dim3(nlong), dim3(64), 0, ks, b->d_order_long + b->long_off[k], b->d_jobs, b->d_tb, b->d_res, b->d_nc, b->d_cig, b->d_err);
+		if (nlong < nk) hipLaunchKernelGGL(ksw_backtrack_kernel, dim3((nk + 63) / 64), dim3(64), 0, ks, nk, b->d_order + off, b->wave_rows, b->d_jobs, b->d_tb, b->d_res, b->d_nc, b->d_cig, b->d_err);
 	}
 	for (int si = 0; si < 4; ++si)
 		if (used_mask >> si & 1) { HIPCHK(hipEventRecord(c->kev[si], side[si])); HIPCHK(hipStreamWaitEvent(c->stream, c->kev[si], 0)); }
 	HIPCHK(hipEventRecord(c->ev[1], c->stream));
-	if (getenv("WM_KSW_COOP_BT") && atoi(getenv("WM_KSW_COOP_BT")) > 0)
-		hipLaunchKernelGGL(ksw_backtrack_coop_kernel, dim3(n), dim3(64), 0, c->stream, n, b->d_jobs, b->d_tb, b->d_res, b->d_cig, b->d_err);
-	else
-		hipLaunchKernelGGL(ksw_backtrack_kernel, dim3((n + 63) / 64), dim3(64), 0, c->stream, n, b->d_jobs, b->d_tb, b->d_res, b->d_cig, b->d_err);
-	hipLaunchKernelGGL(ksw_scan_kernel, dim3(1), dim3(1024), 0, c->stream, n, b->d_res, b->d_off, b->d_total);
-	hipLaunchKernelGGL(ksw_gather_kernel, dim3(n), dim3(64), 0, c->stream, b->d_jobs, b->d_res, b->d_off, b->d_cig, b->d_pool, (uint32_t)b->pool_cap);
+	ksw_scan_launch(c->stream, n, b->d_nc, b->d_wsum, b->d_off, b->d_total);
+	hipLaunchKernelGGL(ksw_gather_kernel, dim3(n), dim3(64), 0, c->stream, b->d_jobs, b->d_nc, b->d_off, b->d_cig, b->d_pool, (uint32_t)b->pool_cap);
 	if (b->d_zd) hipLaunchKernelGGL(ksw_zdwalk_kernel, dim3((n + 63) / 64), dim3(64), 0, c->stream, n, b->sc_in, b->d_jobs, b->d_res, b->d_off, b->d_pool, b->d_seqs, b->d_zd);
 	HIPCHK(hipEventRecord(c->ev[2], c->stream));
 	HIPCHK(hipGetLastError());
-	int *h_small = c->pin_small ? c->pin_small : &b->h_err;
-	uint32_t *h_total = c->pin_small ? (uint32_t*)(c->pin_small + 1) : &b->total_ops;
-	if (c->pin_small) HIPCHK(hipMemcpyAsync(h_small, b->d_err, 8, hipMemcpyDeviceToHost, c->stream));
-	else { HIPCHK(hipMemcpyAsync(h_small, b->d_err, 4, hipMemcpyDeviceToHost, c->stream)); HIPCHK(hipMemcpyAsync(h_total, b->d_total, 4, hipMemcpyDeviceToHost, c->stream)); }
+	HIPCHK(hipMemcpyAsync(b->back.p, b->d_res, b->back_bytes, hipMemcpyDeviceToHost, c->stream));
 	HIPCHK(ctx_sync(c));
-	b->h_err = *h_small; b->total_ops = *h_total;
+	b->h_err = *(const int*)(b->back.p + b->o_err); b->total_ops = *(const uint32_t*)(b->back.p + b->o_err + 4);
 	for (const std::string &f : b->dumped) unlink(f.c_str());
 	b->dumped.clear();
 	HIPCHK(hipEventElapsedTime(&b->dp_ms, c->ev[0], c->ev[1]));
@@ -794,14 +872,13 @@
 	const int n = b->n_jobs;
 	if (cigar_used) *cigar_used = b->total_ops;
 	if (n == 0) return WM_OK;
-	const size_t off_at = (size_t)((uint8_t*)b->d_off - (uint8_t*)b->d_res);
-	UBuf<uint8_t> ro(off_at + (size_t)n * 4, c);
-	const wm_ksw_dres_t *res = (const wm_ksw_dres_t*)ro.data();
-	const uint32_t *off = (const uint32_t*)(ro.data() + off_at);
+	const wm_ksw_dres_t *res = (const wm_ksw_dres_t*)b->back.p;
+	const uint32_t *off = (const uint32_t*)(b->back.p + b->o_off);
 	if (b->total_ops > cigar_cap) return set_err(WM_ENOMEM, "cigar_pool too small: need %u ops", b->total_ops);
-	HIPCHK(hipMemcpyAsync(ro.data(), b->d_res, off_at + (size_t)n * 4, hipMemcpyDeviceToHost, c->stream));
-	if (b->total_ops) HIPCHK(hipMemcpyAsync(cigar_pool, b->d_pool, (size_t)b->total_ops * 4, hipMemcpyDeviceToHost, c->stream));
-	HIPCHK(ctx_sync(c));
+	if (b->total_ops) {
+		HIPCHK(hipMemcpyAsync(cigar_pool, b->d_pool, (size_t)b->total_ops * 4, hipMemcpyDeviceToHost, c->stream));
+		HIPCHK(ctx_sync(c));
+	}
 	WM_SITE("ksw.results");
 	wm::parallel_for(c->host_threads, (size_t)n, [&](size_t i) {
 		wm_ksw_result_t &o = results[i];
@@ -834,11 +911,8 @@
 	const int n = b->n_jobs;
 	if (!b->d_zd) { for (int i = 0; i < n; ++i) out[i] = wm_zd_t{ 0, -1, -1, -1, -1 }; return WM_OK; }
 	if (n == 0) return WM_OK;
-	HIPCHK(hipSetDevice(c->device));
-	UBuf<wm_zd_t> z(n, c);
-	HIPCHK(hipMemcpyAsync(z.data(), b->d_zd, (size_t)n * sizeof(wm_zd_t), hipMemcpyDeviceToHost, c->stream));
-	HIPCHK(ctx_sync(c));
-	memcpy(out, z.data(), (size_t)n * sizeof(wm_zd_t));
+	(void)c;
+	memcpy(out, b->back.p + b->o_zd, (size_t)n * sizeof(wm_zd_t));
 	return WM_OK;
 }
 
@@ -856,7 +930,7 @@
 		while (i1 < n_jobs) {
 			const int ql = pos ? pos[i1].qlen : jobs[i1].qlen, tl = pos ? pos[i1].tlen : jobs[i1].tlen, w = pos ? pos[i1].w : jobs[i1].w;
 			size_t t = 128;
-			if (ql > 0 && tl > 0) t = ((size_t)ql + tl) * ((size_t)wm_ksw_ncol(ql, tl, w) + 10) + 512;
+			if (ql > 0 && tl > 0) t = ((size_t)ql + tl) * ((size_t)wm_ksw_ncol(ql, tl, w) + 10) + 512 + chain_mail_bytes(ql, tl, w, pos ? pos[i1].flag : jobs[i1].flag);
 			if (i1 > i0 && need + t > budget) break;
 			need += t; ++i1;
 		}
@@ -946,7 +1020,7 @@
 	wmk::ksw_dp_exts2<true>(sc, noncan, junc_bonus, jb, seqs, junc, tb, mem, (int*)(mem + 8 * T), res + j);
 }
 __global__ __launch_bounds__(64) void ksw_exts2_backtrack_kernel(wm_ksw_score_t sc, int n, const wm_ksw_djob_t *__restrict__ jobs, const uint8_t *__restrict__ tb,
-                                                                  wm_ksw_dres_t *__restrict__ res, uint32_t *__restrict__ cig_scratch, int *__restrict__ err)
+                                                                  wm_ksw_dres_t *__restrict__ res, uint32_t *__restrict__ ncig, uint32_t *__restrict__ cig_scratch, int *__restrict__ err)
 {
 	const int j = blockIdx.x * 64 + threadIdx.x;
 	if (j >= n) return;
@@ -958,6 +1032,7 @@
 		if (nc < 0) { atomicMax(err, 1); nc = 0; }
 	}
 	res[j].n_cigar = nc;
+	ncig[j] = (uint32_t)nc;
 }
 
 extern "C" int wm_ksw_exts2_batch(wm_ctx_t *c, const wm_ksw_score_t *sc_in, int noncan, int junc_bonus, int n_jobs, const wm_ksw_job_t *jobs,
@@ -1002,13 +1077,14 @@
 	uint32_t *d_off = (uint32_t*)arena_take(c, nj * 4 + 64);
 	uint32_t *d_total = (uint32_t*)arena_take(c, 64);
 	int *d_err = (int*)arena_take(c, 64);
+	uint32_t *d_nc = (uint32_t*)arena_take(c, nj * 4 + 64), *d_wsum = (uint32_t*)arena_take(c, (size_t)ksw_scan_waves(n_jobs) * 4 + 64);
 	uint8_t *d_seqs = (uint8_t*)arena_take(c, seqs_bytes + 64);
 	uint8_t *d_junc = junc ? (uint8_t*)arena_take(c, seqs_bytes + 64) : 0;
 	uint32_t *d_cig = (uint32_t*)arena_take(c, (cig_off + 16) * 4);
 	uint32_t *d_pool = (uint32_t*)arena_take(c, (cig_off + 16) * 4);
 	uint8_t *d_scratch = (uint8_t*)arena_take(c, sc_off + 256);
 	uint8_t *d_tb = (uint8_t*)arena_take(c, tb_off + 64);
-	if (!d_jobs || !d_soff || !d_res || !d_off || !d_total || !d_err || !d_seqs || (junc && !d_junc) || !d_cig || !d_pool || !d_scratch || !d_tb)
+	if (!d_jobs || !d_soff || !d_res || !d_off || !d_total || !d_err || !d_nc || !d_wsum || !d_seqs || (junc && !d_junc) || !d_cig || !d_pool || !d_scratch || !d_tb)
 		return set_err(WM_ENOMEM, "ksw_exts2: batch does not fit the arena (%llu traceback bytes); split it", (unsigned long long)tb_off);
 	HIPCHK(hipMemcpyAsync(d_jobs, dj.data(), nj * sizeof(wm_ksw_djob_t), hipMemcpyHostToDevice, c->stream));
 	HIPCHK(hipMemcpyAsync(d_soff, soff.data(), nj * 8, hipMemcpyHostToDevice, c->stream));
@@ -1016,9 +1092,9 @@
 	if (junc) HIPCHK(hipMemcpyAsync(d_junc, junc, seqs_bytes, hipMemcpyHostToDevice, c->stream));
 	HIPCHK(hipMemsetAsync(d_err, 0, 4, c->stream));
 	hipLaunchKernelGGL(ksw_exts2_kernel, dim3(n_jobs), dim3(64), 0, c->stream, sc, noncan, junc_bonus, d_jobs, d_seqs, d_junc, d_tb, d_scratch, d_soff, d_res);
-	hipLaunchKernelGGL(ksw_exts2_backtrack_kernel, dim3((n_jobs + 63) / 64), dim3(64), 0, c->stream, sc, n_jobs, d_jobs, d_tb, d_res, d_cig, d_err);
-	hipLaunchKernelGGL(ksw_scan_kernel, dim3(1), dim3(1024), 0, c->stream, n_jobs, d_res, d_off, d_total);
-	hipLaunchKernelGGL(ksw_gather_kernel, dim3(n_jobs), dim3(64), 0, c->stream, d_jobs, d_res, d_off, d_cig, d_pool, (uint32_t)(cig_off + 16));
+	hipLaunchKernelGGL(ksw_exts2_backtrack_kernel, dim3((n_jobs + 63) / 64), dim3(64), 0, c->stream, sc, n_jobs, d_jobs, d_tb, d_res, d_nc, d_cig, d_err);
+	ksw_scan_launch(c->stream, n_jobs, d_nc, d_wsum, d_off, d_total);
+	hipLaunchKernelGGL(ksw_gather_kernel, dim3(n_jobs), dim3(64), 0, c->stream, d_jobs, d_nc, d_off, d_cig, d_pool, (uint32_t)(cig_off + 16));
 	HIPCHK(hipGetLastError());
 	UBuf<wm_ksw_dres_t> res(nj, c);
 	UBuf<uint32_t> off(nj, c);
diff --git a/winnowmap_amd/gpu.py b/winnowmap_amd/gpu.py
--- a/winnowmap_amd/gpu.py
+++ b/winnowmap_amd/gpu.py
@@ -51,6 +51,17 @@
     return _lib
 
 
+_bt_walk_env = [None]
+
+
+def _sync_bt_walk():
+    e = os.environ.get("WM_KSW_COOP_BT", "")
+    if e != _bt_walk_env[0]:
+        if _bt_walk_env[0] is not None or e:
+            set_ksw_bt_walk((1 if int(e) > 0 else 0) if e else -1)
+        _bt_walk_env[0] = e
+
+
 def _chk(rc):
     if rc != 0:
         raise WmError("libwmgpu error %d: %s" % (rc, lib().wm_last_error().decode()))
@@ -80,6 +91,7 @@
         cap = int((jobs["qlen"].astype(np.int64) + jobs["tlen"] + 2).sum()) + 16
         pool = np.zeros(cap, np.uint32)
         used = C.c_size_t(0)
+        _sync_bt_walk()
         _chk(lib().wm_ksw_batch(self._h, C.byref(score), len(jobs), jobs.ctypes.data, seqs.ctypes.data, seqs.nbytes,
                                 res.ctypes.data, pool.ctypes.data, cap, C.byref(used)))
         return res, pool[:used.value]
@@ -111,6 +123,7 @@
         cap = int((np.maximum(jobs["qlen"], 0).astype(np.int64) + np.maximum(jobs["tlen"], 0) + 2).sum()) + 16
         pool = np.zeros(cap, np.uint32)
         used = C.c_size_t(0)
+        _sync_bt_walk()
         lib().wm_ksw_batch_pos.argtypes = [C.c_void_p, C.POINTER(KswScore), C.c_int, C.c_void_p, C.c_void_p, C.c_void_p, C.c_size_t, C.POINTER(C.c_size_t)]
         _chk(lib().wm_ksw_batch_pos(self._h, C.byref(score), len(jobs), jobs.ctypes.data, res.ctypes.data, pool.ctypes.data, cap, C.byref(used)))
         return res, pool[:used.value]
@@ -122,6 +135,7 @@
         pool = np.zeros(cap, np.uint32)
         zd = np.zeros((len(jobs), 5), np.int32)
         used = C.c_size_t(0)
+        _sync_bt_walk()
         lib().wm_ksw_batch_pos_zd.argtypes = [C.c_void_p, C.POINTER(KswScore), C.c_int, C.c_void_p, C.c_void_p, C.c_void_p, C.c_size_t, C.POINTER(C.c_size_t), C.c_void_p]
         _chk(lib().wm_ksw_batch_pos_zd(self._h, C.byref(score), len(jobs), jobs.ctypes.data, res.ctypes.data, pool.ctypes.data, cap, C.byref(used), zd.ctypes.data))
         return res, pool[:used.value], zd
@@ -159,6 +173,7 @@
         jobs = np.ascontiguousarray(jobs, KSW_JOB_DTYPE)
         seqs = np.ascontiguousarray(seqs, np.uint8)
         h = C.c_void_p()
+        _sync_bt_walk()
         _chk(lib().wm_ksw_dev_prepare(self._h, C.byref(score), len(jobs), jobs.ctypes.data, seqs.ctypes.data, seqs.nbytes, C.byref(h)))
         return KswDevBatch(self, h, jobs)
 
@@ -199,6 +214,12 @@
     lib().wm_ksw_set_chain_routing.argtypes = [C.c_int, C.c_int, C.c_int]
     lib().wm_ksw_set_chain_routing.restype = None
     lib().wm_ksw_set_chain_routing(mode, min_rows_exact, bp)
+
+
+def set_ksw_bt_walk(mode=-1):
+    lib().wm_ksw_set_bt_walk.argtypes = [C.c_int]
+    lib().wm_ksw_set_bt_walk.restype = None
+    lib().wm_ksw_set_bt_walk(int(mode))
 
 
 def set_ksw_dual(on):
```

Measured after the change: 0.1411. 15.2% lower.
